# dome272/Paella

Hardware: AMD Instinct MI355X
Metric: images/sec (whole node) + single-image ms, 256x256 @ 8 steps (higher is better)
Workload: dtype f32; 1 GPU; BASELINE configs[1]: Paella 573M-class (stand-in blocks=[4,8,4]) (570.3M params), 32x32 tokens = 256 px, 8 steps, CFG 8.0, CLIP-H-text only (S=4), batch 1 per GPU, + VQGAN f8 decode; denoiser=570m, sample_steps=8, noise=philox, submission=hip-graph replay, world_size_observed=1

## Files before the change

include/paella_hip.h:

```cpp
#ifndef PAELLA_HIP_H
#define PAELLA_HIP_H

#include <stddef.h>
#include <stdint.h>

#ifdef __cplusplus
extern "C" {
#endif

#define PAELLA_ABI_VERSION 8

#define PAELLA_OK 0
#define PAELLA_ERR_ARG -1
#define PAELLA_ERR_HIP -2
#define PAELLA_ERR_WORKSPACE -3
#define PAELLA_ERR_STATE -4

#define PAELLA_MAX_LEVELS 8
#define PAELLA_MAX_BLOCK_TYPES 8

int paella_abi_version(void);
const char* paella_last_error(void);
const char* paella_source_stamp(void);

// ... 161 lines not shown
                                         const int* kw_len, int kw_pitch, const int* q_groups, int qg_pitch, const int* k_groups,
                                         int kg_pitch, const uint64_t* seeds, const float* temperature, int rows_per_sample,
                                         const int* step, const float* t_next, const int* active, const int64_t* init_noise,
                                         const int64_t* pin_keep, const int64_t* pin_tokens, const int* pin_on, int64_t* tokens_out,
                                         void* ws, size_t ws_bytes, void* stream);

int paella_sample_tail_filter(const float* logits_c, const float* logits_u, int64_t rows, int L, float cfg, float one_minus_cfg,
                              float temperature, int mode, uint64_t seed, const uint64_t* seed_ptr, uint64_t offset, int64_t row_offset,
                              const int64_t* row_offset_ptr, const int64_t* init_noise, float t_next, const int64_t* pin_keep,
                              const int64_t* pin_tokens, int top_k, float top_p, float typical_mass, int min_tokens,
                              int64_t* tokens_out, int64_t* sampled_out, void* stream);
int paella_sample_tail_stream_filter(const float* logits_c, const float* logits_u, int64_t rows, int L, const float* cfg_pairs,
                                     const float* temperature, const uint64_t* seeds, int rows_per_sample, const int* step,
                                     const float* t_next, const int* active, const int64_t* init_noise, const int64_t* pin_keep,
                                     const int64_t* pin_tokens, const int* pin_on, const int* filter_k, const float* filter_mass,
                                     int64_t* tokens_out, int64_t* sampled_out, void* stream);

int paella_sample_tail_stats(const float* logits_c, const float* logits_u, int64_t rows, int L, float cfg, float one_minus_cfg,
                             float temperature, int mode, uint64_t seed, const uint64_t* seed_ptr, uint64_t offset, int64_t row_offset,
                             const int64_t* row_offset_ptr, const int64_t* init_noise, float t_next, const int64_t* pin_keep,
                             const int64_t* pin_tokens, int top_k, float top_p, float typical_mass, int min_tokens, int64_t* tokens_out,
                             int64_t* sampled_out, float* logprob_out, float* entropy_out, void* stream);
int paella_sample_tail_stream_stats(const float* logits_c, const float* logits_u, int64_t rows, int L, const float* cfg_pairs,
                                    const float* temperature, const uint64_t* seeds, int rows_per_sample, const int* step,
                                    const float* t_next, const int* active, const int64_t* init_noise, const int64_t* pin_keep,
                                    const int64_t* pin_tokens, const int* pin_on, const int* filter_k, const float* filter_mass,
                                    int64_t* tokens_out, int64_t* sampled_out, float* logprob_out, float* entropy_out, void* stream);
int paella_renoise_select(const int64_t* drawn, const float* logprob, const int64_t* init_noise, int64_t rows, int rows_per_sample,
                          uint64_t seed, const uint64_t* seed_ptr, uint64_t offset, int64_t row_offset, const int64_t* row_offset_ptr,
                          float t_next, int policy, float confidence_noise, const int64_t* pin_keep, const int64_t* pin_tokens,
                          int64_t* tokens_out, void* stream);
int paella_renoise_select_stream(const int64_t* drawn, const float* logprob, const int64_t* init_noise, int64_t rows, int rows_per_sample,
                                 const uint64_t* seeds, const int* step, const float* t_next, const int* active, const int* policy,
                                 const float* confidence_noise, const int64_t* pin_keep, const int64_t* pin_tokens, const int* pin_on,
                                 int64_t* tokens_out, void* stream);

typedef struct paella_tail_args {
    const float *logits_c, *logits_u; int64_t rows; int32_t L;
    float cfg, one_minus_cfg, temperature; int32_t mode; uint64_t seed; const uint64_t* seed_ptr; uint64_t offset;
    int64_t row_offset; const int64_t* row_offset_ptr; float t_next; const float *noise_q, *mask_u;
    const uint64_t* seeds; const float *temperature_tab, *cfg_pairs; int32_t rows_per_sample;
    const int32_t* step; const float* t_next_tab; const int32_t* active;
    const int64_t *init_noise, *pin_keep, *pin_tokens; const int32_t* pin_on;
    int32_t top_k; float top_p, typical_mass; int32_t min_tokens; const int32_t* filter_k; const float* filter_mass;
    int64_t *tokens_out, *sampled_out; float *logprob_out, *entropy_out;
} paella_tail_args;

typedef struct paella_step_args {
    const int64_t* tokens; const float* r; const void* cond; int32_t B, n_unique; float mix_c, mix_u; const float* mix_pairs; int32_t H, W, S; const int32_t* cond_len;
    const float* attn_weights; int32_t n_attn_weights;
    const float* kw_table; const int32_t* kw_len; int32_t kw_pitch;
    const int32_t* q_groups; int32_t qg_pitch; const int32_t* k_groups; int32_t kg_pitch;
    float* logits_out; const paella_tail_args* tail;
} paella_step_args;

int paella_unet_step(paella_unet* m, const paella_step_args* args, size_t args_bytes, void* ws, size_t ws_bytes, void* stream);
int paella_sample_tail_args(const paella_tail_args* args, size_t args_bytes, void* stream);

int paella_add_noise(const int64_t* x, const float* t, const int64_t* mask_in, const int64_t* random_x,
                     const float* rand_u, uint64_t seed, uint64_t offset, int num_labels, int B,
                     int64_t per_sample, int64_t* x_out, int64_t* mask_out, void* stream);

int paella_select_tokens(const int64_t* a, const int64_t* b, const int64_t* mask, const float* flag, int64_t fill, int64_t n,
                         int64_t* out, void* stream);

typedef struct paella_vqgan paella_vqgan;
typedef struct paella_vqgan_config {
    int32_t levels, bottleneck_blocks, c_hidden, c_latent, codebook_size;
    float scale_factor;
} paella_vqgan_config;

int paella_vqgan_create(const paella_vqgan_config* cfg, paella_vqgan** out);
void paella_vqgan_destroy(paella_vqgan* v);
int paella_vqgan_load_tensor(paella_vqgan* v, const char* key, const float* dev_src, const int64_t* shape, int ndim,
                             void* stream);
int paella_vqgan_finalize(paella_vqgan* v, void* stream);
int paella_vqgan_set_precision(paella_vqgan* v, int mode, void* stream);
size_t paella_vqgan_workspace_bytes(const paella_vqgan* v, int B, int h, int w);
int paella_vqgan_decode_indices(paella_vqgan* v, const int64_t* idx, int B, int h, int w, float* img_out, void* ws,
                                size_t ws_bytes, void* stream);
int paella_vqgan_decode(paella_vqgan* v, const float* latents, int B, int h, int w, float* img_out, void* ws,
                        size_t ws_bytes, void* stream);
int paella_vqgan_encode(paella_vqgan* v, const float* img, int B, int Hp, int Wp, float* qe_out, float* x_out,
                        int64_t* idx_out, float* loss_out, void* ws, size_t ws_bytes, void* stream);
int paella_vqgan_quantize_rows(paella_vqgan* v, const float* x, int64_t rows, int64_t* idx_out, float* qe_out,
                               float* mse_out, void* stream);
int paella_vqgan_lookup_rows(paella_vqgan* v, const int64_t* idx, int64_t rows, float* out, void* stream);

int paella_op_gemm(const float* A, const float* W, const float* bias, const float* residual, float* C, int M, int N,
                   int K, int act, int tile_cfg, int splitk, void* ws, size_t ws_bytes, void* stream);
int paella_op_layernorm(const float* x, float* y, int64_t rows, int C, float eps, void* stream);
int paella_op_dwconv_ln(const float* x, const float* skip, const float* w, const float* bias, float* y, int B, int H,
                        int W, int C, float eps, void* stream);
int paella_op_grn_scale(const float* g, const float* gamma, float* scale, float* tmp, int B, int rows_per_sample,
                        int C, void* stream);
int paella_op_attention(const float* q, const float* k_self, const float* v_self, const float* k_cond,
                        const float* v_cond, float* out, int B, int nhead, int D, int Lq, int Lself, int Lcond,
                        const float* key_weights, int n_kw, void* stream);
int paella_op_attention_ragged(const float* q, const float* k_self, const float* v_self, const float* k_cond,
                               const float* v_cond, float* out, int B, int nhead, int D, int Lq, int Lself, int Lcond,
                               const int* cond_len, const float* key_weights, int n_kw, void* stream);
int paella_op_attention_kw(const float* q, const float* k_self, const float* v_self, const float* k_cond, const float* v_cond,
                           float* out, int B, int nhead, int D, int Lq, int Lself, int Lcond, const int* cond_len,
                           const float* kw_table, const int* kw_len, int kw_pitch, void* stream);
int paella_op_attention_rg(const float* q, const float* k_self, const float* v_self, const float* k_cond, const float* v_cond,
                           float* out, int B, int nhead, int D, int Lq, int Lself, int Lcond, const int* cond_len,
                           const float* kw_table, const int* kw_len, int kw_pitch, const int* q_groups, int qg_pitch,
// ... 109 lines not shown
```

paella_amd/_lib.py:

```python
import ctypes
import os
from ctypes import POINTER, Structure, c_char, c_char_p, c_double, c_float, c_int, c_int32, c_int64, c_size_t, c_uint64, c_void_p

_HERE = os.path.dirname(os.path.abspath(__file__))
LIB_PATH = os.path.join(_HERE, "csrc", "libpaella_hip.so")

MAX_LEVELS = 8
MAX_BLOCK_TYPES = 8
ABI_VERSION = 8


class UnetConfig(Structure):
    _fields_ = [
        ("c_in", c_int32), ("c_out", c_int32), ("num_labels", c_int32), ("c_r", c_int32), ("patch_size", c_int32),
        ("c_cond", c_int32), ("n_levels", c_int32),
        ("c_hidden", c_int32 * MAX_LEVELS), ("nhead", c_int32 * MAX_LEVELS), ("blocks", c_int32 * MAX_LEVELS),
        ("level_config", (c_char * MAX_BLOCK_TYPES) * MAX_LEVELS),
        ("clip_embd", c_int32), ("byt5_embd", c_int32), ("clip_seq_len", c_int32), ("kernel_size", c_int32),
        ("self_attn", c_int32),
    ]


class VqganConfig(Structure):
    _fields_ = [
        ("levels", c_int32), ("bottleneck_blocks", c_int32), ("c_hidden", c_int32), ("c_latent", c_int32),
        ("codebook_size", c_int32), ("scale_factor", c_float),
    ]


class TestGemmArgs(Structure):
    _fields_ = [
        ("A", c_void_p), ("lda", c_int), ("W", c_void_p), ("ldw", c_int), ("C", c_void_p), ("ldc", c_int),
        ("M", c_int), ("N", c_int), ("K", c_int),
        ("bias", c_void_p), ("act", c_int), ("alpha", c_float), ("residual", c_void_p), ("ldr", c_int),
        ("ts", c_void_p), ("ts_stride", c_int), ("rows_per_sample", c_int),
        ("store_mode", c_int), ("sH", c_int), ("sW", c_int), ("sC", c_int), ("py", c_int), ("px", c_int), ("n_seg_x", c_int),
        ("rowstat_out", c_void_p), ("sumsq_out", c_void_p),
        ("remap_in", c_int), ("remap_out", c_int), ("remap_off", c_int),
        ("c16", c_void_p),
        ("mode", c_int), ("scale", c_void_p), ("shift", c_void_p), ("a_rows_per_sample", c_int), ("ln_stats", c_void_p),
        ("cv_enabled", c_int), ("cv_Hi", c_int), ("cv_Wi", c_int), ("cv_C", c_int), ("cv_Ho", c_int), ("cv_Wo", c_int), ("cv_stride", c_int),
        ("cv_ntaps", c_int), ("cv_tw_log2", c_int), ("cv_oy0", c_int), ("cv_ox0", c_int), ("cv_tsign", c_int),
        ("c_capacity", c_size_t), ("c16_capacity", c_size_t), ("rowstat_capacity", c_size_t), ("sumsq_capacity", c_size_t),
    ]


class TailArgs(Structure):
    _fields_ = [
        ("logits_c", c_void_p), ("logits_u", c_void_p), ("rows", c_int64), ("L", c_int32),
        ("cfg", c_float), ("one_minus_cfg", c_float), ("temperature", c_float), ("mode", c_int32), ("seed", c_uint64), ("seed_ptr", c_void_p), ("offset", c_uint64),
        ("row_offset", c_int64), ("row_offset_ptr", c_void_p), ("t_next", c_float), ("noise_q", c_void_p), ("mask_u", c_void_p),
        ("seeds", c_void_p), ("temperature_tab", c_void_p), ("cfg_pairs", c_void_p), ("rows_per_sample", c_int32),
        ("step", c_void_p), ("t_next_tab", c_void_p), ("active", c_void_p),
        ("init_noise", c_void_p), ("pin_keep", c_void_p), ("pin_tokens", c_void_p), ("pin_on", c_void_p),
        ("top_k", c_int32), ("top_p", c_float), ("typical_mass", c_float), ("min_tokens", c_int32), ("filter_k", c_void_p), ("filter_mass", c_void_p),
        ("tokens_out", c_void_p), ("sampled_out", c_void_p), ("logprob_out", c_void_p), ("entropy_out", c_void_p),
    ]


class StepArgs(Structure):
    _fields_ = [
        ("tokens", c_void_p), ("r", c_void_p), ("cond", c_void_p), ("B", c_int32), ("n_unique", c_int32), ("mix_c", c_float), ("mix_u", c_float), ("mix_pairs", c_void_p),
        ("H", c_int32), ("W", c_int32), ("S", c_int32), ("cond_len", c_void_p),
        ("attn_weights", c_void_p), ("n_attn_weights", c_int32),
        ("kw_table", c_void_p), ("kw_len", c_void_p), ("kw_pitch", c_int32),
        ("q_groups", c_void_p), ("qg_pitch", c_int32), ("k_groups", c_void_p), ("kg_pitch", c_int32),
        ("logits_out", c_void_p), ("tail", POINTER(TailArgs)),
    ]


class AdamwTensor(Structure):
    _fields_ = [
        ("p", c_void_p), ("g", c_void_p), ("m", c_void_p), ("v", c_void_p), ("n", c_int64), ("chunk_begin", c_int64),
        ("lr", c_double), ("beta1", c_double), ("beta2", c_double), ("eps", c_double), ("weight_decay", c_double),
    ]


def tensor_fields(block, **tensors):
    for name, t in tensors.items():
        setattr(block, name, None if t is None else t.data_ptr())
    return block


SIGNATURES = {
    "paella_abi_version": (c_int, []),
    "paella_last_error": (c_char_p, []),
    "paella_source_stamp": (c_char_p, []),
    "paella_workspace_init": (c_int, [c_void_p, c_size_t, c_void_p]),
    "paella_workspace_header_bytes": (c_size_t, []),
    "paella_unet_create": (c_int, [POINTER(UnetConfig), POINTER(c_void_p)]),
    "paella_unet_destroy": (None, [c_void_p]),
    "paella_unet_load_tensor": (c_int, [c_void_p, c_char_p, c_void_p, POINTER(c_int64), c_int, c_void_p]),
    "paella_unet_set_timestep_freqs": (c_int, [c_void_p, POINTER(c_float), c_int]),
    "paella_unet_finalize": (c_int, [c_void_p, c_void_p]),
    "paella_unet_cond_bytes": (c_size_t, [c_void_p, c_int, c_int]),
    "paella_unet_workspace_bytes": (c_size_t, [c_void_p, c_int, c_int, c_int, c_int]),
    "paella_unet_cond_prepare": (c_int, [c_void_p, c_void_p, c_int, c_void_p, POINTER(c_void_p), c_int, c_int, c_void_p,
                                         c_size_t, c_void_p, c_size_t, c_void_p]),
    "paella_unet_c_embeddings": (c_int, [c_void_p, c_void_p, c_int, c_void_p, POINTER(c_void_p), c_int, c_int, c_void_p,
                                         c_void_p, c_size_t, c_void_p]),
    "paella_unet_r_embedding": (c_int, [c_void_p, c_void_p, c_int, c_float, c_void_p, c_void_p]),
    "paella_unet_forward": (c_int, [c_void_p, c_void_p, c_void_p, c_void_p, c_int, c_int, c_int, c_int, c_void_p, c_int,
                                    c_void_p, c_void_p, c_size_t, c_void_p]),
    "paella_unet_forward_shared": (c_int, [c_void_p, c_void_p, c_void_p, c_void_p, c_int, c_int, c_float, c_float, c_int, c_int, c_int,
                                           c_void_p, c_int, c_void_p, c_void_p, c_size_t, c_void_p]),
    "paella_unet_forward_sample": (c_int, [c_void_p, c_void_p, c_void_p, c_void_p, c_int, c_int, c_float, c_float, c_int, c_int, c_int,
                                           c_void_p, c_int, c_float, c_int, c_uint64, c_void_p, c_uint64, c_int64, c_void_p, c_void_p, c_float, c_void_p,
                                           c_void_p, c_size_t, c_void_p]),
    "paella_sample_tail": (c_int, [c_void_p, c_void_p, c_int64, c_int, c_float, c_float, c_float, c_int, c_void_p,
                                   c_uint64, c_uint64, c_void_p, c_void_p, c_float, c_void_p, c_void_p, c_void_p]),
    "paella_sample_tail_ex": (c_int, [c_void_p, c_void_p, c_int64, c_int, c_float, c_float, c_float, c_int, c_void_p,
                                      c_uint64, c_void_p, c_uint64, c_int64, c_void_p, c_void_p, c_void_p, c_float, c_void_p, c_void_p, c_void_p]),
    "paella_start_tokens": (c_int, [c_uint64, c_void_p, c_int64, c_void_p, c_int, c_int64, c_void_p, c_void_p]),
    "paella_sample_tail_req": (c_int, [c_void_p, c_void_p, c_int64, c_int, c_void_p, c_void_p, c_void_p, c_int, c_uint64, c_void_p, c_float, c_void_p, c_void_p,
                                       c_void_p]),
    "paella_start_tokens_req": (c_int, [c_void_p, c_int, c_int, c_int, c_void_p, c_void_p]),
    "paella_unet_forward_shared_req": (c_int, [c_void_p, c_void_p, c_void_p, c_void_p, c_int, c_int, c_void_p, c_int, c_int, c_int, c_void_p, c_int, c_void_p,
                                               c_void_p, c_size_t, c_void_p]),
    "paella_unet_forward_sample_req": (c_int, [c_void_p, c_void_p, c_void_p, c_void_p, c_int, c_int, c_void_p, c_int, c_int, c_int, c_void_p, c_int, c_void_p,
                                               c_void_p, c_int, c_uint64, c_void_p, c_float, c_void_p, c_void_p, c_size_t, c_void_p]),
    "paella_request_step": (c_int, [c_void_p, c_int, c_void_p, c_void_p, c_int, c_void_p, c_void_p, c_void_p, c_void_p, c_void_p, c_void_p, c_void_p]),
    "paella_sample_tail_stream": (c_int, [c_void_p, c_void_p, c_int64, c_int, c_void_p, c_void_p, c_void_p, c_int, c_void_p, c_void_p, c_void_p, c_void_p, c_void_p,
                                          c_void_p, c_void_p]),
    "paella_unet_forward_sample_stream": (c_int, [c_void_p, c_void_p, c_void_p, c_void_p, c_int, c_int, c_void_p, c_int, c_int, c_int, c_void_p, c_int, c_void_p,
                                                  c_void_p, c_int, c_void_p, c_void_p, c_void_p, c_void_p, c_void_p, c_void_p, c_size_t, c_void_p]),
    "paella_add_noise": (c_int, [c_void_p, c_void_p, c_void_p, c_void_p, c_void_p, c_uint64, c_uint64, c_int, c_int,
                                 c_int64, c_void_p, c_void_p, c_void_p]),
    "paella_select_tokens": (c_int, [c_void_p, c_void_p, c_void_p, c_void_p, c_int64, c_int64, c_void_p, c_void_p]),
    "paella_vqgan_create": (c_int, [POINTER(VqganConfig), POINTER(c_void_p)]),
    "paella_vqgan_destroy": (None, [c_void_p]),
    "paella_vqgan_load_tensor": (c_int, [c_void_p, c_char_p, c_void_p, POINTER(c_int64), c_int, c_void_p]),
    "paella_vqgan_finalize": (c_int, [c_void_p, c_void_p]),
    "paella_vqgan_set_precision": (c_int, [c_void_p, c_int, c_void_p]),
    "paella_vqgan_workspace_bytes": (c_size_t, [c_void_p, c_int, c_int, c_int]),
    "paella_vqgan_decode_indices": (c_int, [c_void_p, c_void_p, c_int, c_int, c_int, c_void_p, c_void_p, c_size_t, c_void_p]),
    "paella_vqgan_decode": (c_int, [c_void_p, c_void_p, c_int, c_int, c_int, c_void_p, c_void_p, c_size_t, c_void_p]),
    "paella_vqgan_encode": (c_int, [c_void_p, c_void_p, c_int, c_int, c_int, c_void_p, c_void_p, c_void_p, c_void_p,
                                    c_void_p, c_size_t, c_void_p]),
    "paella_vqgan_quantize_rows": (c_int, [c_void_p, c_void_p, c_int64, c_void_p, c_void_p, c_void_p, c_void_p]),
    "paella_vqgan_lookup_rows": (c_int, [c_void_p, c_void_p, c_int64, c_void_p, c_void_p]),
    "paella_unet_set_precision": (c_int, [c_void_p, c_int, c_void_p]),
    "paella_unet_get_precision": (c_int, [c_void_p]),
    "paella_op_gemm": (c_int, [c_void_p, c_void_p, c_void_p, c_void_p, c_void_p, c_int, c_int, c_int, c_int, c_int, c_int,
                               c_void_p, c_size_t, c_void_p]),
    "paella_op_layernorm": (c_int, [c_void_p, c_void_p, c_int64, c_int, c_float, c_void_p]),
    "paella_op_dwconv_ln": (c_int, [c_void_p, c_void_p, c_void_p, c_void_p, c_void_p, c_int, c_int, c_int, c_int, c_float,
                                    c_void_p]),
    "paella_op_grn_scale": (c_int, [c_void_p, c_void_p, c_void_p, c_void_p, c_int, c_int, c_int, c_void_p]),
    "paella_op_attention": (c_int, [c_void_p, c_void_p, c_void_p, c_void_p, c_void_p, c_void_p, c_int, c_int, c_int, c_int,
                                    c_int, c_int, c_void_p, c_int, c_void_p]),
    "paella_unet_cond_prepare_slots": (c_int, [c_void_p, c_void_p, c_int, c_void_p, POINTER(c_void_p), c_int, c_int, c_int, c_int, c_void_p,
                                               c_size_t, c_void_p, c_void_p, c_size_t, c_void_p]),
    "paella_unet_forward_shared_ragged": (c_int, [c_void_p, c_void_p, c_void_p, c_void_p, c_int, c_int, c_float, c_float, c_int, c_int, c_int, c_void_p,
                                                  c_void_p, c_int, c_void_p, c_void_p, c_size_t, c_void_p]),
# ... 86 lines not shown
    "paella_grn_act_forward_seed_dev": (c_int, [c_void_p, c_void_p, c_void_p, c_int, c_int, c_int, c_float, c_void_p, c_void_p, c_void_p, c_void_p, c_size_t, c_void_p]),
    "paella_grn_act_backward_seed_dev": (c_int, [c_void_p, c_void_p, c_void_p, c_void_p, c_int, c_int, c_int, c_float, c_void_p, c_void_p, c_void_p, c_void_p, c_void_p,
                                                 c_size_t, c_void_p]),
    "paella_attn_train_forward_seed_dev": (c_int, [c_void_p, c_int, c_void_p, c_int, c_void_p, c_int, c_int, c_int, c_int, c_int, c_int, c_float, c_void_p, c_void_p,
                                                   c_void_p, c_void_p, c_size_t, c_void_p]),
    "paella_attn_train_backward_seed_dev": (c_int, [c_void_p, c_int, c_void_p, c_int, c_void_p, c_int, c_void_p, c_void_p, c_void_p, c_int, c_int, c_int, c_int, c_int,
                                                    c_float, c_void_p, c_void_p, c_int, c_void_p, c_int, c_void_p, c_int, c_void_p, c_size_t, c_void_p]),
    "paella_embed_ln_train_workspace_bytes": (c_size_t, [c_int, c_int, c_int, c_int, c_int, c_int]),
    "paella_embed_ln_train_forward": (c_int, [c_void_p, c_void_p, c_int, c_int, c_int, c_int, c_int, c_int, c_float, c_void_p, c_void_p, c_size_t, c_void_p]),
    "paella_embed_ln_train_backward": (c_int, [c_void_p, c_void_p, c_void_p, c_int, c_int, c_int, c_int, c_int, c_int, c_float, c_void_p, c_void_p, c_size_t, c_void_p]),
}

TEST_HOOKS = {
    "paella_prof_detail": (c_int64, [c_void_p, c_void_p, c_int64]),
    "paella_prof_epi": (c_int64, [c_void_p, c_int64]),
    "paella_prof_grid": (c_int64, [c_void_p, c_int64]),
    "paella_prof_enable": (c_int, [c_int]),
    "paella_prof_collect": (c_int, [POINTER(ctypes.c_double), POINTER(ctypes.c_double), POINTER(ctypes.c_double), POINTER(c_int64)]),
    "paella_test_gemm_bf16": (c_int, [c_void_p, c_void_p, c_void_p, c_void_p, c_void_p, c_void_p, c_int, c_int, c_int, c_int, c_void_p, c_int, c_int, c_void_p, c_size_t, c_void_p]),
    "paella_test_gemm_bf16_rule": (c_int, [c_int]),
    "paella_test_grn_apply16": (c_int, [c_void_p, c_void_p, c_void_p, c_int64, c_int, c_int, c_void_p]),
    "paella_test_gemm_bf16_ln": (c_int, [c_void_p, c_void_p, c_void_p, c_void_p, c_int, c_int, c_int, c_void_p, c_int, c_int, c_void_p, c_size_t, c_void_p]),
    "paella_test_attention_bf16": (c_int, [c_void_p, c_void_p, c_void_p, c_void_p, c_void_p, c_void_p, c_int, c_int, c_int, c_int, c_int, c_int, c_void_p, c_int, c_void_p]),
    "paella_test_attention_bf16_ragged": (c_int, [c_void_p, c_void_p, c_void_p, c_void_p, c_void_p, c_void_p, c_int, c_int, c_int, c_int, c_int, c_int, c_void_p,
                                                  c_void_p, c_int, c_void_p]),
    "paella_test_attention_bf16_kw": (c_int, [c_void_p, c_void_p, c_void_p, c_void_p, c_void_p, c_void_p, c_int, c_int, c_int, c_int, c_int, c_int, c_void_p,
                                              c_void_p, c_void_p, c_int, c_void_p]),
    "paella_test_launch_chain": (c_int, [c_void_p, c_int, c_int, c_int, c_void_p]),
    "paella_test_attention_variant": (c_int, [c_int]),
    "paella_test_gemm_dma": (c_int, [c_int]),
    "paella_test_gemm_epi_specialise": (c_int, [c_int]),
    "paella_test_gemm_raster": (c_int, [c_int]),
    "paella_test_gemm_ring": (c_int, [c_int]),
    "paella_test_ring_resident": (ctypes.c_long, [c_int, c_int]),
    "paella_test_gemm_site": (c_int, [c_int, c_int, c_int, c_int, c_int, c_int]),
    "paella_test_gemm_site_cfg": (c_int, [c_int, c_int, c_int, c_int, c_int, c_int, c_int]),
    "paella_test_gemm_big_stagger": (c_int, [c_int]),
    "paella_test_grn_fuse": (c_int, [c_int]),
    "paella_test_ln_fold_ratio": (c_int, [c_float]),
    "paella_test_ln_guard_counter": (c_int, [c_void_p]),
    "paella_test_mlp_grn_fused": (c_int, [c_void_p] * 10 + [c_int, c_int, c_int, c_void_p, c_size_t, c_void_p]),
    "paella_test_gemm_tail_tile": (c_int, [c_int]),
    "paella_test_tail_scores": (c_int, [c_void_p, c_void_p, c_int64, c_int, c_float, c_float, c_float, c_uint64, c_uint64, c_int64, c_void_p, c_void_p]),
    "paella_test_tail_scores_req": (c_int, [c_void_p, c_void_p, c_int64, c_int, c_void_p, c_void_p, c_void_p, c_int, c_uint64, c_void_p, c_void_p]),
    "paella_test_tail_filter_keep": (c_int, [c_void_p, c_void_p, c_int64, c_int, c_float, c_float, c_float, c_int, c_float, c_float, c_int, c_void_p, c_void_p, c_void_p,
                                             c_int, c_void_p, c_void_p, c_void_p, c_void_p, c_void_p]),
    "paella_test_renoise_scores": (c_int, [c_void_p, c_void_p, c_void_p, c_int64, c_int, c_uint64, c_uint64, c_int64, c_float, c_int, c_float, c_void_p, c_void_p, c_void_p,
                                           c_void_p, c_void_p, c_void_p, c_void_p, c_void_p, c_void_p, c_void_p, c_void_p, c_void_p]),
    "paella_test_gemm_prologue": (c_int, [c_void_p, c_void_p, c_void_p, c_int, c_int, c_int, c_int, c_void_p, c_void_p, c_int, c_void_p, c_int, c_int,
                                          c_void_p, c_size_t, c_void_p]),
    "paella_test_gemm_desc": (c_int, [POINTER(TestGemmArgs), c_int, c_int, c_void_p, c_size_t, c_void_p]),
    "paella_test_gemm_args_size": (c_size_t, []),
    "paella_test_embed_ln_unshuffle": (c_int, [c_void_p, c_void_p, c_void_p, c_int, c_int, c_int, c_int, c_int, c_int, c_float, c_void_p]),
}

_lib = None


class PaellaHipError(RuntimeError):
    pass


def load():
    global _lib
    if _lib is not None:
        return _lib
    if not os.path.exists(LIB_PATH):
        raise PaellaHipError(
            "libpaella_hip.so is not built (%s). Run `python -m paella_amd.build` (needs hipcc); "
            "paella_amd has no non-HIP fallback." % LIB_PATH)
    try:
        lib = ctypes.CDLL(LIB_PATH)
    except OSError as e:
        raise PaellaHipError("cannot load %s: %s" % (LIB_PATH, e)) from e
    for name, (res, args) in list(SIGNATURES.items()) + list(TEST_HOOKS.items()):
        fn = getattr(lib, name)
        fn.restype = res
        fn.argtypes = args
    from ._stamp import source_stamp
    try:
        here = source_stamp()
    except OSError as e:
        raise PaellaHipError("cannot verify %s: the kernel sources it is checked against are missing (%s)" % (LIB_PATH, e)) from e
    built = lib.paella_source_stamp().decode()
    if built != here:
        raise PaellaHipError("libpaella_hip.so was built from other sources (library stamp %s, sources in the tree %s): rebuild with "
                             "`python -m paella_amd.build`; a stale library is never used silently" % (built, here))
    if lib.paella_abi_version() != ABI_VERSION:
        raise PaellaHipError("libpaella_hip.so ABI %d != binding ABI %d" % (lib.paella_abi_version(), ABI_VERSION))
    _lib = lib
    return lib


def check(rc):
    if rc != 0:
        msg = load().paella_last_error()
        raise PaellaHipError("libpaella_hip error %d: %s" % (rc, msg.decode("utf-8", "replace") if msg else "?"))


def ptr(t):
    return None if t is None else c_void_p(t.data_ptr())


def new_workspace(nbytes, device):
    import torch
    lib = load()
# ... 11 lines not shown
```

paella_amd/csrc/common.h:

```cpp
#pragma once
#include <hip/hip_runtime.h>
#include <stdint.h>
#include <stddef.h>

typedef float f32x4 __attribute__((ext_vector_type(4)));

#define PAELLA_OK 0
#define PAELLA_ERR_ARG -1
#define PAELLA_ERR_HIP -2
#define PAELLA_ERR_WORKSPACE -3
#define PAELLA_ERR_STATE -4

void paella_set_error(const char* fmt, ...);

#define HIP_CHECK_RET(expr)                                                          \
    do {                                                                             \
        hipError_t _e = (expr);                                                      \
        if (_e != hipSuccess) {                                                      \
            paella_set_error("%s:%d: %s -> %s", __FILE__, __LINE__, #expr,           \
                             hipGetErrorString(_e));                                 \
            return PAELLA_ERR_HIP;                                                   \
        }                                                                            \
    } while (0)

// ... 89 lines not shown
    int Hi, Wi, C, Ho, Wo, stride, ntaps;
    int tw_log2, oy0, ox0, tsign;
};

struct GemmArgs {
    const float* A; int lda;
    const float* W; int ldw;
    float* C; int ldc;
    int M, N, K;
    const float* a_scale;
    const float* a_shift;
    int a_rows_per_sample;
    FastDiv a_rps_div;
    const float* grn_gx;
    const float* grn_gamma;
    const float* grn_part;
    int grn_np;
    int force_ring_cfg;
    const float* ln_stats;
    int ln_nblk;
    float ln_eps;
    const float* ln_row;
    float ln_fold_ratio;
    const float* ln_wsum;
    unsigned* ln_guard_count;
    Epilogue ep;
    FusedTail ft;
    ConvGather cv;
    const unsigned short* A16;
    const unsigned short* W16;
    ReqTables rq;
};

struct TailArgs;
static const size_t kGemmMaxTickets = (size_t)1 << 16;
static const size_t kGemmTicketBytes = kGemmMaxTickets * sizeof(unsigned);
int launch_gemm(const GemmArgs& g, void* ws, size_t ws_bytes, hipStream_t stream);
int launch_gemm_cfg(const GemmArgs& g, int cfg, int splitk, void* ws, size_t ws_bytes, hipStream_t stream);
int gemm_num_tile_configs();
int gemm_grn_fused_tile(int M, int C4, int C, int rows_per_sample, bool allow_64);
int gemm_tail_tiles_n(int M, int N, bool bf16_operands = false);
int launch_gemm_tail(const GemmArgs& g, hipStream_t stream);
int gemm_tail_config(int M, int N, bool bf16_operands = false);
int launch_tail_finalize(const TailArgs& a, const float* part_score, const int* part_idx, int tiles_n, hipStream_t stream);
static inline bool gemm_bf16_ok(int K, int lda, int ldw) { return K > 0 && (K & 63) == 0 && (lda & 7) == 0 && (ldw & 7) == 0; }

int launch_ln_rowstat_finalize(const float* stats, int nblk, int K, float eps, float* out4, int64_t M, const float* A32, unsigned short* A16, int lda, float ratio,
                               unsigned* guard_count, hipStream_t stream);

int launch_layernorm(const float* x, float* y, int64_t rows, int C, float eps, float g_mul, float g_add,
                     int s2d, int H, int W, hipStream_t stream);
int launch_layernorm16(const float* x, float* y, unsigned short* y16, int64_t rows, int C, float eps, float g_mul, float g_add,
                       int s2d, int H, int W, hipStream_t stream);
int launch_grn_apply16(unsigned short* h, const float* scale, const float* shift, int64_t rows, int rows_per_sample, int C, hipStream_t stream);
int launch_grn_partials_apply16(const float* part, const float* gamma, const float* shift, float* scale, unsigned short* h, int B, int rows_per_sample, int C, hipStream_t stream);
int launch_f32_to_bf16(const float* src, unsigned short* dst, size_t n, hipStream_t stream);
int launch_rowsum_bf16(const unsigned short* W, float* out, int N, int K, hipStream_t stream);

int launch_dwconv_ln(const float* x, const float* skip, const float* w, const float* bias, float* y,
                     int B, int H, int W, int C, float eps, hipStream_t stream, unsigned short* y16 = nullptr);
int launch_dwconv_res(const float* x, const float* xt, const float* w, const float* bias, float* y,
                      int B, int H, int W, int C, float gamma2, hipStream_t stream);

int launch_grn_scale(const float* g, const float* gamma, float* scale, float* tmp_gx, int B,
                     int rows_per_sample, int C, hipStream_t stream);

int launch_grn_from_partials(const float* part, const float* gamma, float* scale, int B, int groups, int C, hipStream_t stream);

int launch_embed_ln_unshuffle(const int64_t* tokens, const float* table, float* out, int B, int H, int W,
                              int c_in, int patch, int num_labels, float eps, hipStream_t stream);

int launch_timestep(const float* r, const float* freqs, const float* Wcat, const float* bcat, float* ts,
                    int B, int c_r, int total, float max_positions, float* r_embed_out, int reps, hipStream_t stream);
int launch_scale_shift(float* x, const float* ts, int ts_stride, int64_t rows, int rows_per_sample, int C,
                       hipStream_t stream);

int launch_silu(const float* x, float* y, int64_t n, hipStream_t stream);
int launch_copy_rows(const float* src, int lds, float* dst, int ldd, int64_t rows, int cols, hipStream_t stream);
int launch_axpby(float* x, const float* y, float a, float b, int64_t n, hipStream_t stream);
int launch_axpby16(float* x, const float* y, float a, float b, int64_t n, unsigned short* x16, hipStream_t stream);
int launch_axpby16_req(float* x, const float* y, const float* ab, int B, int64_t per_sample, unsigned short* x16, hipStream_t stream);

struct AttnArgs {
    const float* q; int ldq;
    const float* k_self; const float* v_self; int ld_self;
    const float* k_cond; const float* v_cond; int ld_cond;
    float* out; int ldo;
    int B, nhead, D, Lq, Lself, Lcond;
    float scale;
    const float* key_weights;
    int n_kw;
    unsigned short* out16;
    const unsigned short* q16; const unsigned short* k_self16; const unsigned short* v_self16; int ld16;
    const int* cond_len;
    const float* kw_table = nullptr;
    const int* kw_len = nullptr;
    int kw_pitch = 0;
    const int* q_groups = nullptr;
    const int* k_groups = nullptr;
    int qg_pitch = 0, kg_pitch = 0;
};
int launch_attention(const AttnArgs& a, hipStream_t stream);

struct TailArgs {
    const float* logits_c; const float* logits_u;
    int64_t rows; int L;
    float cfg, one_minus_cfg, temperature;
    int mode;
    const float* noise_q;
    uint64_t seed; uint64_t offset;
    int64_t row_offset;
    const uint64_t* seed_ptr;
    const int64_t* row_offset_ptr;
    const int64_t* init_noise;
    const float* mask_u;
    float t_next;
    int64_t* tokens_out;
    int64_t* sampled_out;
    ReqTables rq;
    const int64_t* pin_keep = nullptr;
    const int64_t* pin_tokens = nullptr;
    const int* pin_on = nullptr;
};
int launch_sample_tail(const TailArgs& a, hipStream_t stream);
struct TailFilter {
    int top_k = 0, min_tokens = 1;
    float top_p = 1.f, typical_mass = 1.f;
    const int* filter_k = nullptr;
    const float* filter_mass = nullptr;
    unsigned char* keep_out = nullptr;
    float* rec_out = nullptr;
// ... 42 lines not shown
```

paella_amd/csrc/elementwise.hip:

```cpp
#include "common.h"
#include "gemm_device.h"

#define WAVES_PER_BLOCK 4

__device__ __forceinline__ float wave_sum(float v) {
#pragma unroll
    for (int o = 32; o > 0; o >>= 1) v += __shfl_xor(v, o, 64);
    return v;
}

__device__ __forceinline__ f32x4 ld4(const float* p) { return *reinterpret_cast<const f32x4*>(p); }
__device__ __forceinline__ void st4(float* p, f32x4 v) { *reinterpret_cast<f32x4*>(p) = v; }
__device__ __forceinline__ float hsum4(f32x4 v) { return (v[0] + v[1]) + (v[2] + v[3]); }
typedef __bf16 bf16x4 __attribute__((ext_vector_type(4)));
typedef __bf16 bf16x8 __attribute__((ext_vector_type(8)));
typedef float f32x8 __attribute__((ext_vector_type(8)));
__device__ __forceinline__ void st4h(unsigned short* p, f32x4 v) { *reinterpret_cast<bf16x4*>(p) = __builtin_convertvector(v, bf16x4); }

template <int NV>
__device__ __forceinline__ void ln_regs(f32x4 (&v)[NV], int C4, int lane, int C, float eps, float mul, float add) {
    float s = 0.f;
#pragma unroll
    for (int i = 0; i < NV; ++i)
        if (lane + i * 64 < C4) s += hsum4(v[i]);
// ... 29 lines not shown
    }
    ln_regs<NV>(v, C4, lane, C, eps, g_mul, g_add);
    int64_t yo;
    if (s2d) {
        const int64_t hw = (int64_t)H * W;
        const int64_t b = row / hw;
        const int rem = (int)(row - b * hw);
        const int yy = rem / W, xx = rem - yy * W;
        const int64_t orow = (b * (H >> 1) + (yy >> 1)) * (W >> 1) + (xx >> 1);
        yo = orow * (4 * (int64_t)C) + ((yy & 1) * 2 + (xx & 1)) * C;
    } else {
        yo = row * C;
    }
    if (y16) {
#pragma unroll
        for (int i = 0; i < NV; ++i) {
            const int c4 = lane + i * 64;
            if (c4 < C4) st4h(y16 + yo + c4 * 4, v[i]);
        }
    }
    if (y) {
#pragma unroll
        for (int i = 0; i < NV; ++i) {
            const int c4 = lane + i * 64;
            if (c4 < C4) st4(y + yo + c4 * 4, v[i]);
        }
    }
}

#define DISPATCH_NV(C4, ...)                                                       \
    do {                                                                           \
        const int _nv = ((C4) + 63) / 64;                                          \
        if (_nv <= 1) { constexpr int NV = 1; __VA_ARGS__; }                       \
        else if (_nv <= 2) { constexpr int NV = 2; __VA_ARGS__; }                  \
        else if (_nv <= 3) { constexpr int NV = 3; __VA_ARGS__; }                  \
        else if (_nv <= 5) { constexpr int NV = 5; __VA_ARGS__; }                  \
        else if (_nv <= 8) { constexpr int NV = 8; __VA_ARGS__; }                  \
        else if (_nv <= 16) { constexpr int NV = 16; __VA_ARGS__; }                \
        else { paella_set_error("channel count %d too large", (C4) * 4); return PAELLA_ERR_ARG; } \
    } while (0)

int launch_layernorm(const float* x, float* y, int64_t rows, int C, float eps, float g_mul, float g_add, int s2d,
                     int H, int W, hipStream_t st) {
    return launch_layernorm16(x, y, nullptr, rows, C, eps, g_mul, g_add, s2d, H, W, st);
}
int launch_layernorm16(const float* x, float* y, unsigned short* y16, int64_t rows, int C, float eps, float g_mul, float g_add, int s2d,
                       int H, int W, hipStream_t st) {
    if (rows <= 0) return PAELLA_OK;
    if (C & 3) { paella_set_error("layernorm: C %% 4 != 0 (C=%d)", C); return PAELLA_ERR_ARG; }
    if (s2d && ((H & 1) || (W & 1))) { paella_set_error("layernorm s2d: odd grid %dx%d", H, W); return PAELLA_ERR_ARG; }
    const unsigned blocks = (unsigned)((rows + WAVES_PER_BLOCK - 1) / WAVES_PER_BLOCK);
    DISPATCH_NV(C >> 2, hipLaunchKernelGGL((layernorm_kernel<NV>), dim3(blocks), dim3(64 * WAVES_PER_BLOCK), 0, st, x, y, y16,
                                           rows, C, eps, g_mul, g_add, s2d, H, W));
    LAUNCH_CHECK_RET();
    return PAELLA_OK;
}

__global__ __launch_bounds__(256) void ln_rowstat_finalize_kernel(const float* __restrict__ stats, int nblk, int K, float eps, f32x4* __restrict__ out, int64_t M,
                                                                  const float* __restrict__ A32, unsigned short* __restrict__ A16, int lda, float ratio,
                                                                  unsigned* __restrict__ guard_count) {
    const int64_t row = (int64_t)blockIdx.x * 16 + (threadIdx.x >> 4);
    const int l16 = threadIdx.x & 15;
    if (row >= M) return;
    const float* st = stats + (size_t)row * nblk * 2;
    RowStatAcc acc;
    for (int j = l16; j < nblk; j += 16) acc.add(st[2 * j], st[2 * j + 1]);
#pragma unroll
    for (int o = 1; o < 16; o <<= 1) { acc.S += __shfl_xor(acc.S, o, 64); acc.Q += __shfl_xor(acc.Q, o, 64); acc.M += __shfl_xor(acc.M, o, 64); }
    float mu, rs;
    acc.finish(K, eps, mu, rs);
    const float mu_lo = (float)(acc.S / (double)K - (double)mu);
    if (l16 == 0) out[row] = f32x4{mu, rs, mu_lo, fabsf(mu) * rs};
    if (A16 && fabsf(mu) * rs > ratio) {
        typedef __bf16 bf16x4_t __attribute__((ext_vector_type(4)));
        const float* src = A32 + (size_t)row * lda;
        unsigned short* dst = A16 + (size_t)row * lda;
        for (int k = l16 * 4; k < K; k += 64) {
            f32x4 v = *reinterpret_cast<const f32x4*>(src + k);
#pragma unroll
            for (int e = 0; e < 4; ++e) v[e] = ((v[e] - mu) - mu_lo) * rs;
            *reinterpret_cast<bf16x4_t*>(dst + k) = __builtin_convertvector(v, bf16x4_t);
        }
        if (guard_count && l16 == 0) atomicAdd(guard_count, 1u);
    }
}

int launch_ln_rowstat_finalize(const float* stats, int nblk, int K, float eps, float* out4, int64_t M, const float* A32, unsigned short* A16, int lda, float ratio,
                               unsigned* guard_count, hipStream_t st) {
    if (M <= 0) return PAELLA_OK;
    if (A16 && (!A32 || (K & 3) || (lda & 3))) { paella_set_error("ln_rowstat_finalize: the bf16 rewrite needs the fp32 rows and K, lda %% 4 == 0"); return PAELLA_ERR_ARG; }
    hipLaunchKernelGGL(ln_rowstat_finalize_kernel, dim3((unsigned)((M + 15) / 16)), dim3(256), 0, st, stats, nblk, K, eps, reinterpret_cast<f32x4*>(out4), M, A32, A16, lda, ratio,
                       guard_count);
    LAUNCH_CHECK_RET();
    return PAELLA_OK;
}


template <int NV>
__global__ __launch_bounds__(64 * WAVES_PER_BLOCK) void dwconv_res_kernel(const float* __restrict__ x,
                                                                         const float* __restrict__ xt,
                                                                         const float* __restrict__ w,
                                                                         const float* __restrict__ bias,
                                                                         float* __restrict__ y, int B, int H, int W, int C,
                                                                         float gamma2) {
    const int lane = threadIdx.x & 63;
    const int64_t pos = (int64_t)blockIdx.x * WAVES_PER_BLOCK + (threadIdx.x >> 6);
    const int64_t total = (int64_t)B * H * W;
    if (pos >= total) return;
    const int C4 = C >> 2;
    const int xx = (int)(pos % W);
    const int yy = (int)((pos / W) % H);
    const int64_t base = pos - (int64_t)yy * W - xx;
    f32x4 acc[NV];
#pragma unroll
    for (int i = 0; i < NV; ++i) {
        const int c4 = lane + i * 64;
        acc[i] = c4 < C4 ? ld4(bias + c4 * 4) : f32x4{0.f, 0.f, 0.f, 0.f};
    }
#pragma unroll
    for (int ky = 0; ky < 3; ++ky) {
        const int sy = min(max(yy + ky - 1, 0), H - 1);
#pragma unroll
        for (int kx = 0; kx < 3; ++kx) {
            const int sx = min(max(xx + kx - 1, 0), W - 1);
            const int64_t npos = base + (int64_t)sy * W + sx;
            const int tap = ky * 3 + kx;
#pragma unroll
            for (int i = 0; i < NV; ++i) {
                const int c4 = lane + i * 64;
                if (c4 < C4) acc[i] += ld4(xt + npos * C + c4 * 4) * ld4(w + tap * C + c4 * 4);
            }
        }
    }
#pragma unroll
    for (int i = 0; i < NV; ++i) {
        const int c4 = lane + i * 64;
        if (c4 < C4) st4(y + pos * C + c4 * 4, ld4(x + pos * C + c4 * 4) + acc[i] * gamma2);
    }
}

int launch_dwconv_res(const float* x, const float* xt, const float* w, const float* bias, float* y, int B, int H,
                      int W, int C, float gamma2, hipStream_t st) {
    const int64_t total = (int64_t)B * H * W;
    if (total <= 0) return PAELLA_OK;
    if (C & 3) { paella_set_error("dwconv_res: C %% 4 != 0"); return PAELLA_ERR_ARG; }
    const unsigned blocks = (unsigned)((total + WAVES_PER_BLOCK - 1) / WAVES_PER_BLOCK);
    DISPATCH_NV(C >> 2, hipLaunchKernelGGL((dwconv_res_kernel<NV>), dim3(blocks), dim3(64 * WAVES_PER_BLOCK), 0, st, x, xt, w,
                                           bias, y, B, H, W, C, gamma2));
    LAUNCH_CHECK_RET();
    return PAELLA_OK;
}

__global__ __launch_bounds__(256) void grn_sumsq_kernel(const float* __restrict__ g, float* __restrict__ gx, int rows_per_sample,
                                                        int C) {
    __shared__ float red[4][64];
    const int cl = threadIdx.x & 63, rg = threadIdx.x >> 6;
    const int c = blockIdx.x * 64 + cl;
    const int b = blockIdx.y;
    float s = 0.f;
    if (c < C) {
        const float* p = g + ((size_t)b * rows_per_sample) * C + c;
        for (int r = rg; r < rows_per_sample; r += 4) {
            const float v = p[(size_t)r * C];
            s += v * v;
        }
    }
    red[rg][cl] = s;
    __syncthreads();
    if (rg == 0 && c < C) gx[(size_t)b * C + c] = sqrtf((red[0][cl] + red[1][cl]) + (red[2][cl] + red[3][cl]));
}

__global__ __launch_bounds__(256) void grn_finalize_kernel(const float* __restrict__ gx, const float* __restrict__ gamma,
                                                           float* __restrict__ scale, int C) {
    __shared__ float red[256];
    const int b = blockIdx.x;
    const float* p = gx + (size_t)b * C;
    float s = 0.f;
    for (int c = threadIdx.x; c < C; c += 256) s += p[c];
    red[threadIdx.x] = s;
    __syncthreads();
    for (int o = 128; o > 0; o >>= 1) {
        if ((int)threadIdx.x < o) red[threadIdx.x] += red[threadIdx.x + o];
        __syncthreads();
    }
    const float denom = red[0] / (float)C + 1e-6f;
    for (int c = threadIdx.x; c < C; c += 256) scale[(size_t)b * C + c] = 1.0f + gamma[c] * (p[c] / denom);
}

template <int G>
__global__ __launch_bounds__(1024) void grn_from_partials_kernel(const float* __restrict__ part, const float* __restrict__ gamma,
                                                                 float* __restrict__ scale, int groups_rt, int C) {
    __shared__ float red[16];
    const int groups = G > 0 ? G : groups_rt;
    const int b = blockIdx.y;
    const int C4 = C >> 2;
    const float* p = part + (size_t)b * groups * C;
    auto colsum = [&](int c4) {
        f32x4 q = f32x4{0.f, 0.f, 0.f, 0.f};
        if (G > 0) {
            f32x4 v[G > 0 ? G : 1];
#pragma unroll
            for (int g = 0; g < G; ++g) v[g] = ld4(p + (size_t)g * C + c4 * 4);
#pragma unroll
            for (int g = 0; g < G; ++g) q += v[g];
        } else {
// ... 69 lines not shown
#pragma unroll
    for (int t = 0; t < P * P; ++t) {
        const int dy = t / P, dx = t % P;
        int64_t tok = tokens[(b * H + (oy * P + dy)) * W + (ox * P + dx)];
        tok = tok < 0 ? 0 : (tok >= num_labels ? num_labels - 1 : tok);
        const float* row = table + tok * c_in;
        float s = 0.f;
        for (int c4 = lane; c4 < C4; c4 += 64) s += hsum4(ld4(row + c4 * 4));
        const float mean = wave_sum(s) / (float)c_in;
        float q = 0.f;
        for (int c4 = lane; c4 < C4; c4 += 64) {
            f32x4 d = ld4(row + c4 * 4) - mean;
            d = d * d;
            q += hsum4(d);
        }
        const float rstd = 1.0f / sqrtf(wave_sum(q) / (float)c_in + eps);
        for (int c4 = lane; c4 < C4; c4 += 64) {
            const f32x4 n = (ld4(row + c4 * 4) - mean) * rstd;
#pragma unroll
            for (int e = 0; e < 4; ++e) orow[(c4 * 4 + e) * (P * P) + t] = n[e];
        }
    }
}

int launch_embed_ln_unshuffle(const int64_t* tokens, const float* table, float* out, int B, int H, int W, int c_in,
                              int patch, int num_labels, float eps, hipStream_t st) {
    if (c_in & 3) { paella_set_error("embed: c_in %% 4 != 0"); return PAELLA_ERR_ARG; }
    if (patch < 1 || patch > 2 || (H % patch) || (W % patch)) {
        paella_set_error("embed: unsupported patch_size %d for grid %dx%d (supported: 1, 2)", patch, H, W);
        return PAELLA_ERR_ARG;
    }
    const int64_t total = (int64_t)B * (H / patch) * (W / patch);
    if (total <= 0) return PAELLA_OK;
    if (total > 0x7fffffff) { paella_set_error("embed: too many positions"); return PAELLA_ERR_ARG; }
    const unsigned blocks = (unsigned)((total + WAVES_PER_BLOCK - 1) / WAVES_PER_BLOCK);
    const FastDiv dWo = fast_div_of((unsigned)(W / patch)), dHo = fast_div_of((unsigned)(H / patch));
    if (patch == 2)
        hipLaunchKernelGGL((embed_ln_unshuffle_kernel<2>), dim3(blocks), dim3(64 * WAVES_PER_BLOCK), 0, st, tokens, table, out,
                           B, H, W, c_in, num_labels, eps, dWo, dHo);
    else
        hipLaunchKernelGGL((embed_ln_unshuffle_kernel<1>), dim3(blocks), dim3(64 * WAVES_PER_BLOCK), 0, st, tokens, table, out,
                           B, H, W, c_in, num_labels, eps, dWo, dHo);
    LAUNCH_CHECK_RET();
    return PAELLA_OK;
}

__global__ __launch_bounds__(256) void timestep_kernel(const float* __restrict__ r, const float* __restrict__ freqs,
                                                       const float* __restrict__ Wcat, const float* __restrict__ bcat,
                                                       float* __restrict__ ts, int c_r, int total, float max_positions,
                                                       float* __restrict__ r_embed_out, int reps, int n_distinct) {
    extern __shared__ float emb[];
    const int b = blockIdx.y;
    const int half = c_r >> 1;
    const float rr = r[b] * max_positions;
    for (int k = threadIdx.x; k < c_r; k += 256) {
        float v = 0.f;
        if (k < half) v = sinf(rr * freqs[k]);
        else if (k < 2 * half) v = cosf(rr * freqs[k - half]);
        emb[k] = v;
        if (r_embed_out && blockIdx.x == 0) r_embed_out[(size_t)b * c_r + k] = v;
    }
    __syncthreads();
    const int o = blockIdx.x * 256 + threadIdx.x;
    if (o >= total) return;
    const float* w = Wcat + (size_t)o * c_r;
    float acc = 0.f;
    for (int k = 0; k < c_r; ++k) acc += emb[k] * w[k];
    const float out = acc + bcat[o];
    for (int rep = 0; rep < reps; ++rep) ts[((size_t)rep * n_distinct + b) * total + o] = out;
}

int launch_timestep(const float* r, const float* freqs, const float* Wcat, const float* bcat, float* ts, int B,
                    int c_r, int total, float max_positions, float* r_embed_out, int reps, hipStream_t st) {
    if (B <= 0) return PAELLA_OK;
    int gx = (total + 255) / 256;
    if (gx < 1) gx = 1;
    hipLaunchKernelGGL(timestep_kernel, dim3(gx, B), dim3(256), c_r * sizeof(float), st, r, freqs, Wcat, bcat, ts, c_r,
                       total, max_positions, r_embed_out, reps < 1 ? 1 : reps, B);
    LAUNCH_CHECK_RET();
    return PAELLA_OK;
}

__global__ __launch_bounds__(256) void scale_shift_kernel(float* __restrict__ x, const float* __restrict__ ts, int ts_stride,
                                                          int64_t rows, int rows_per_sample, int C) {
    const int C4 = C >> 2;
    const int64_t total = rows * C4;
    for (int64_t i = (int64_t)blockIdx.x * 256 + threadIdx.x; i < total; i += (int64_t)gridDim.x * 256) {
        const int64_t row = i / C4;
        const int c = (int)(i - row * C4) * 4;
        const float* t = ts + (row / rows_per_sample) * ts_stride;
        const f32x4 v = ld4(x + row * C + c);
        st4(x + row * C + c, v * (1.0f + ld4(t + c)) + ld4(t + C + c));
    }
}

int launch_scale_shift(float* x, const float* ts, int ts_stride, int64_t rows, int rows_per_sample, int C,
                       hipStream_t st) {
    if (rows <= 0) return PAELLA_OK;
    if (C & 3) { paella_set_error("scale_shift: C %% 4 != 0"); return PAELLA_ERR_ARG; }
    int64_t blocks = (rows * (C >> 2) + 255) / 256;
    if (blocks > 4096) blocks = 4096;
    hipLaunchKernelGGL(scale_shift_kernel, dim3((unsigned)blocks), dim3(256), 0, st, x, ts, ts_stride, rows, rows_per_sample, C);
    LAUNCH_CHECK_RET();
    return PAELLA_OK;
}

__global__ __launch_bounds__(256) void silu_kernel(const float* __restrict__ x, float* __restrict__ y, int64_t n) {
    for (int64_t i = (int64_t)blockIdx.x * 256 + threadIdx.x; i < n; i += (int64_t)gridDim.x * 256) {
        const float v = x[i];
        y[i] = v / (1.0f + expf(-v));
    }
}
int launch_silu(const float* x, float* y, int64_t n, hipStream_t st) {
    if (n <= 0) return PAELLA_OK;
    int64_t blocks = (n + 255) / 256;
    if (blocks > 4096) blocks = 4096;
    hipLaunchKernelGGL(silu_kernel, dim3((unsigned)blocks), dim3(256), 0, st, x, y, n);
    LAUNCH_CHECK_RET();
    return PAELLA_OK;
}

__global__ __launch_bounds__(256) void copy_rows_kernel(const float* __restrict__ src, int lds_, float* __restrict__ dst, int ldd,
                                                        int64_t rows, int cols) {
    const int64_t total = rows * cols;
    for (int64_t i = (int64_t)blockIdx.x * 256 + threadIdx.x; i < total; i += (int64_t)gridDim.x * 256) {
        const int64_t r = i / cols;
        const int c = (int)(i - r * cols);
        dst[r * ldd + c] = src[r * lds_ + c];
    }
}
__global__ __launch_bounds__(256) void copy_rows4_kernel(const float* __restrict__ src, int lds_, float* __restrict__ dst, int ldd, unsigned total4, int cols4, FastDiv dC) {
    for (unsigned i = blockIdx.x * 256u + threadIdx.x; i < total4; i += gridDim.x * 256u) {
        const unsigned r = fast_div(i, dC);
        const unsigned c = (i - r * (unsigned)cols4) * 4u;
        st4(dst + (size_t)r * ldd + c, ld4(src + (size_t)r * lds_ + c));
    }
}
__global__ __launch_bounds__(256) void axpby_kernel(float* __restrict__ x, const float* __restrict__ y, float a, float b, int64_t n4, unsigned short* __restrict__ x16) {
    for (int64_t i = (int64_t)blockIdx.x * 256 + threadIdx.x; i < n4; i += (int64_t)gridDim.x * 256) {
        const f32x4 v = ld4(x + i * 4) * a + ld4(y + i * 4) * b;
        st4(x + i * 4, v);
        if (x16) st4h(x16 + i * 4, v);
    }
}
__global__ __launch_bounds__(256) void axpby_req_kernel(float* __restrict__ x, const float* __restrict__ y, const float* __restrict__ ab, int64_t per4, unsigned short* __restrict__ x16) {
    const int s = blockIdx.y;
    const float a = ab[2 * s], b = ab[2 * s + 1];
    for (int64_t j = (int64_t)blockIdx.x * 256 + threadIdx.x; j < per4; j += (int64_t)gridDim.x * 256) {
        const int64_t i = (int64_t)s * per4 + j;
        const f32x4 v = ld4(x + i * 4) * a + ld4(y + i * 4) * b;
        st4(x + i * 4, v);
        if (x16) st4h(x16 + i * 4, v);
    }
}
int launch_axpby16_req(float* x, const float* y, const float* ab, int B, int64_t per_sample, unsigned short* x16, hipStream_t st) {
    if (B <= 0 || per_sample <= 0) return PAELLA_OK;
    if (!ab || (per_sample & 3) || B > 65535) { paella_set_error("axpby_req: needs a pair table, per_sample %% 4 == 0 and at most 65535 samples"); return PAELLA_ERR_ARG; }
    int64_t blocks = (per_sample / 4 + 255) / 256;
    if (blocks > 1024) blocks = 1024;
    hipLaunchKernelGGL(axpby_req_kernel, dim3((unsigned)blocks, (unsigned)B), dim3(256), 0, st, x, y, ab, per_sample / 4, x16);
    LAUNCH_CHECK_RET();
    return PAELLA_OK;
}
int launch_axpby(float* x, const float* y, float a, float b, int64_t n, hipStream_t st) { return launch_axpby16(x, y, a, b, n, nullptr, st); }
int launch_axpby16(float* x, const float* y, float a, float b, int64_t n, unsigned short* x16, hipStream_t st) {
    if (n <= 0) return PAELLA_OK;
    if (n & 3) { paella_set_error("axpby: n %% 4 != 0"); return PAELLA_ERR_ARG; }
    int64_t blocks = (n / 4 + 255) / 256;
    if (blocks > 8192) blocks = 8192;
    hipLaunchKernelGGL(axpby_kernel, dim3((unsigned)blocks), dim3(256), 0, st, x, y, a, b, n / 4, x16);
    LAUNCH_CHECK_RET();
    return PAELLA_OK;
}

int launch_copy_rows(const float* src, int lds_, float* dst, int ldd, int64_t rows, int cols, hipStream_t st) {
    if (rows <= 0 || cols <= 0) return PAELLA_OK;
    if (!((cols | lds_ | ldd) & 3) && !(((uintptr_t)src | (uintptr_t)dst) & 15) && rows * (cols / 4) < 0x7fffffff) {
        const int64_t total4 = rows * (cols / 4);
        int64_t blocks4 = (total4 + 255) / 256;
        if (blocks4 > 4096) blocks4 = 4096;
        hipLaunchKernelGGL(copy_rows4_kernel, dim3((unsigned)blocks4), dim3(256), 0, st, src, lds_, dst, ldd, (unsigned)total4, cols / 4, fast_div_of((unsigned)(cols / 4)));
        LAUNCH_CHECK_RET();
        return PAELLA_OK;
    }
    int64_t blocks = (rows * cols + 255) / 256;
    if (blocks > 4096) blocks = 4096;
    hipLaunchKernelGGL(copy_rows_kernel, dim3((unsigned)blocks), dim3(256), 0, st, src, lds_, dst, ldd, rows, cols);
    LAUNCH_CHECK_RET();
    return PAELLA_OK;
}

__global__ __launch_bounds__(256) void grn_apply16_kernel(unsigned short* __restrict__ h, const float* __restrict__ scale, const float* __restrict__ shift,
                                                          unsigned total8, int C8, FastDiv dC8, FastDiv dRps) {
    for (unsigned i = blockIdx.x * 256u + threadIdx.x; i < total8; i += gridDim.x * 256u) {
        const unsigned row = fast_div(i, dC8);
        const unsigned c = (i - row * (unsigned)C8) * 8u;
        const unsigned b = fast_div(row, dRps);
        const bf16x8 v = *reinterpret_cast<const bf16x8*>(h + (size_t)i * 8);
        const float* sp = scale + (size_t)b * ((size_t)C8 * 8) + c;
        const f32x4 s0 = ld4(sp), s1 = ld4(sp + 4), t0 = ld4(shift + c), t1 = ld4(shift + c + 4);
        const f32x8 f = __builtin_convertvector(v, f32x8);
        f32x8 o;
#pragma unroll
        for (int e = 0; e < 4; ++e) { o[e] = f[e] * s0[e] + t0[e]; o[4 + e] = f[4 + e] * s1[e] + t1[e]; }
        *reinterpret_cast<bf16x8*>(h + (size_t)i * 8) = __builtin_convertvector(o, bf16x8);
    }
}
__global__ __launch_bounds__(256) void grn_apply16_cols_kernel(unsigned short* __restrict__ h, const float* __restrict__ scale, const float* __restrict__ shift, int C, int rows_per_sample) {
    const int c = (blockIdx.x * 64 + (threadIdx.x & 63)) * 8;
    const int b = blockIdx.z;
    const int r0 = blockIdx.y * 16 + (threadIdx.x >> 6);
    unsigned short* hp = h + ((size_t)b * rows_per_sample + r0) * C + c;
    bf16x8 v[4];
#pragma unroll
    for (int k = 0; k < 4; ++k) v[k] = *reinterpret_cast<const bf16x8*>(hp + (size_t)(4 * k) * C);
    const float* sp = scale + (size_t)b * C + c;
    const f32x4 s0 = ld4(sp), s1 = ld4(sp + 4), t0 = ld4(shift + c), t1 = ld4(shift + c + 4);
#pragma unroll
    for (int k = 0; k < 4; ++k) {
        const f32x8 f = __builtin_convertvector(v[k], f32x8);
        f32x8 o;
#pragma unroll
        for (int e = 0; e < 4; ++e) { o[e] = f[e] * s0[e] + t0[e]; o[4 + e] = f[4 + e] * s1[e] + t1[e]; }
// ... 128 lines not shown
```

paella_amd/csrc/model.hip:

```cpp
#include "internal.h"
#include "test_hooks.h"
#include "../../include/paella_hip.h"

#include <math.h>
#include <stdarg.h>
#include <stdio.h>
#include <string.h>

#include <map>
#include <string>
#include <vector>

static thread_local char g_err[2048] = "";
void paella_set_error(const char* fmt, ...) {
    va_list ap;
    va_start(ap, fmt);
    vsnprintf(g_err, sizeof(g_err), fmt, ap);
    va_end(ap);
}
extern "C" const char* paella_last_error(void) { return g_err; }
extern "C" int paella_abi_version(void) { return PAELLA_ABI_VERSION; }

int devbuf_alloc(DevBuf& b, size_t n) {
    if (b.p && b.n == n) return PAELLA_OK;
    if (b.p) { (void)hipFree(b.p); b.p = nullptr; }
    b.n = n;
    HIP_CHECK_RET(hipMalloc((void**)&b.p, (n ? n : 1) * sizeof(float)));
    return PAELLA_OK;
}

enum BlockType { BT_RES, BT_TS, BT_ATTN, BT_FF, BT_DOWN, BT_UP };

struct Block {
    BlockType type;
    int level = 0;
    int c = 0;
    bool has_skip = false;
    int ts_offset = -1;
    bool ts_standalone = true;
    int fused_ts = -1;
    int attn_index = -1;
    bool emit_rowstat = false;
    bool ln_from_stats = false;
    int c_from = 0, c_to = 0;
    Weight *dw_w = nullptr, *dw_b = nullptr;
    Weight *w1 = nullptr, *b1 = nullptr, *gamma = nullptr, *beta = nullptr, *w2 = nullptr, *b2 = nullptr;
    Weight *in_w = nullptr, *in_b = nullptr, *out_w = nullptr, *out_b = nullptr, *kv_w = nullptr, *kv_b = nullptr;
    Weight *conv_w = nullptr, *conv_b = nullptr;
};

struct LnWeight { Weight* t; int N, K; };

struct paella_unet {
    paella_unet_config cfg;
    std::vector<Block> down, up;
    std::map<std::string, Weight> t;
    Weight *byt5_w, *byt5_b, *clip_w, *clip_b, *clip_image_w, *clip_image_b;
    Weight *in_mapper, *embedding_w, *embedding_b, *clf_w, *clf_b, *out_mapper;
    std::vector<Weight*> shadowed;
    std::vector<LnWeight> ln_weights;
    DevBuf ts_w, ts_b, freqs;
// ... 473 lines not shown
    carve_forward(m, a, B, H, W, S, f);
    Arena c(nullptr, 0);
    carve_cond(m, c, B, S, f);
    return (a.off > c.off ? a.off : c.off) + 256;
}

static int compute_c_embed(const paella_unet* m, const float* byt5, int S_byt5, const float* clip, const float* const* clip_image,
                           int n_clip_image, int B, int S, float* c_embed, float* splitk, hipStream_t st) {
    const paella_unet_config& c = m->cfg;
    const size_t skb = kSplitKBudget;
    const int cc = c.c_cond;
    if (S_byt5 > 0) {
        GemmArgs g = gemm_args(byt5, c.byt5_embd, m->byt5_w->w.p, c.byt5_embd, c_embed, cc, B * S_byt5, cc, c.byt5_embd);
        g.ep.bias = m->byt5_b->w.p;
        g.ep.remap_in = S_byt5; g.ep.remap_out = S; g.ep.remap_off = 0;
        RET_IF(launch_gemm(g, splitk, skb, st));
    }
    int row_off = S_byt5;
    if (clip) {
        GemmArgs g = gemm_args(clip, c.clip_embd, m->clip_w->w.p, c.clip_embd, c_embed + (size_t)row_off * cc, S * cc, B,
                               cc * c.clip_seq_len, c.clip_embd);
        g.ep.bias = m->clip_b->w.p;
        RET_IF(launch_gemm(g, splitk, skb, st));
        row_off += c.clip_seq_len;
    }
    for (int i = 0; i < n_clip_image; ++i) {
        if (!clip_image || !clip_image[i]) { paella_set_error("clip_image[%d] is null", i); return PAELLA_ERR_ARG; }
        GemmArgs g = gemm_args(clip_image[i], c.clip_embd, m->clip_image_w->w.p, c.clip_embd,
                               c_embed + (size_t)row_off * cc, S * cc, B, cc * c.clip_seq_len, c.clip_embd);
        g.ep.bias = m->clip_image_b->w.p;
        RET_IF(launch_gemm(g, splitk, skb, st));
        row_off += c.clip_seq_len;
    }
    RET_IF(launch_layernorm(c_embed, c_embed, (int64_t)B * S, cc, 1e-6f, 1.f, 0.f, 0, 0, 0, st));
    return PAELLA_OK;
}

extern "C" int paella_unet_c_embeddings(paella_unet* m, const float* byt5, int S_byt5, const float* clip,
                                        const float* const* clip_image, int n_clip_image, int B, float* c_embed_out, void* ws,
                                        size_t ws_bytes, void* stream) {
    if (!m || !m->finalized) { paella_set_error("model not finalized"); return PAELLA_ERR_STATE; }
    const int S = S_byt5 + (clip ? m->cfg.clip_seq_len : 0) + n_clip_image * m->cfg.clip_seq_len;
    if (B <= 0 || S <= 0 || !c_embed_out) { paella_set_error("bad conditioning shape"); return PAELLA_ERR_ARG; }
    if (ws_bytes < kSplitKBudget || !ws) { paella_set_error("workspace too small"); return PAELLA_ERR_WORKSPACE; }
    return compute_c_embed(m, byt5, S_byt5, clip, clip_image, n_clip_image, B, S, c_embed_out, (float*)ws, (hipStream_t)stream);
}

extern "C" int paella_unet_r_embedding(paella_unet* m, const float* r, int B, float max_positions, float* r_embed_out, void* stream) {
    if (!m || !m->finalized) { paella_set_error("model not finalized"); return PAELLA_ERR_STATE; }
    if (!r || !r_embed_out) { paella_set_error("null argument"); return PAELLA_ERR_ARG; }
    return launch_timestep(r, m->freqs.p, m->ts_w.p, m->ts_b.p, nullptr, B, m->cfg.c_r, 0, max_positions, r_embed_out, 1, (hipStream_t)stream);
}

static int cond_prepare_impl(paella_unet* m, const float* byt5, int S_byt5, const float* clip, const float* const* clip_image, int n_clip_image, int B,
                             int S_slot, int slot0, void* cond_out, size_t cond_bytes, int* cond_len, void* ws, size_t ws_bytes, void* stream) {
    if (!m || !m->finalized) { paella_set_error("model not finalized"); return PAELLA_ERR_STATE; }
    hipStream_t st = (hipStream_t)stream;
    const paella_unet_config& c = m->cfg;
    const int S = S_byt5 + (clip ? c.clip_seq_len : 0) + n_clip_image * c.clip_seq_len;
    if (B <= 0 || S_byt5 < 0 || n_clip_image < 0) { paella_set_error("bad conditioning shape"); return PAELLA_ERR_ARG; }
    const bool slots = S_slot > 0;
    if (slots && (slot0 < 0 || S > S_slot || !cond_len)) {
        paella_set_error("cond_prepare_slots: %d conditioning rows do not fit a slot of %d rows (or slot0 < 0 / cond_len is null)", S, S_slot);
        return PAELLA_ERR_ARG;
    }
    if (S <= 0 && (slots || m->n_attn > 0)) { paella_set_error("conditioning sequence is empty"); return PAELLA_ERR_ARG; }
    if (slots) HIP_CHECK_RET(hipMemsetD32Async((hipDeviceptr_t)(cond_len + slot0), S, (size_t)B, st));
    if (m->n_attn == 0) return PAELLA_OK;
    if (S_byt5 > 0 && !byt5) { paella_set_error("byt5 is null"); return PAELLA_ERR_ARG; }
    const size_t need = slots ? (size_t)(slot0 + B) * S_slot * (size_t)m->kv_total * sizeof(float) : paella_unet_cond_bytes(m, B, S);
    if (cond_bytes < need || !cond_out) { paella_set_error("cond buffer too small"); return PAELLA_ERR_WORKSPACE; }
    FwdBuffers f;
    Arena a(ws, ws_bytes);
    carve_cond(m, a, B, S, f);
    if (!a.ok || !ws) { paella_set_error("workspace too small (%zu needed)", a.off); return PAELLA_ERR_WORKSPACE; }
    const size_t skb = kSplitKBudget;

    const int cc = c.c_cond;
    RET_IF(compute_c_embed(m, byt5, S_byt5, clip, clip_image, n_clip_image, B, S, f.c_embed, f.splitk, st));
    RET_IF(launch_silu(f.c_embed, f.c_silu, (int64_t)B * S * cc, st));

    GemmArgs g = gemm_args(f.c_silu, cc, m->kv_w.p, cc, (float*)cond_out, m->kv_total, B * S, m->kv_total, cc);
    g.ep.bias = m->kv_b.p;
    if (slots) { g.ep.remap_in = S; g.ep.remap_out = S_slot; g.ep.remap_off = slot0 * S_slot; }
    RET_IF(launch_gemm(g, f.splitk, skb, st));
    return PAELLA_OK;
}

extern "C" int paella_unet_cond_prepare(paella_unet* m, const float* byt5, int S_byt5, const float* clip,
                                        const float* const* clip_image, int n_clip_image, int B, void* cond_out,
                                        size_t cond_bytes, void* ws, size_t ws_bytes, void* stream) {
    return cond_prepare_impl(m, byt5, S_byt5, clip, clip_image, n_clip_image, B, 0, 0, cond_out, cond_bytes, nullptr, ws, ws_bytes, stream);
}

extern "C" int paella_unet_cond_prepare_slots(paella_unet* m, const float* byt5, int S_byt5, const float* clip, const float* const* clip_image,
                                              int n_clip_image, int B, int S_slot, int slot0, void* cache, size_t cache_bytes, int* cond_len, void* ws,
                                              size_t ws_bytes, void* stream) {
    if (S_slot <= 0) { paella_set_error("cond_prepare_slots: S_slot must be > 0"); return PAELLA_ERR_ARG; }
    return cond_prepare_impl(m, byt5, S_byt5, clip, clip_image, n_clip_image, B, S_slot, slot0, cache, cache_bytes, cond_len, ws, ws_bytes, stream);
}

struct FwdCtx {
    const paella_unet* m;
    const paella_step_args& s;
    hipStream_t st;
    FwdBuffers f;
// ... 137 lines not shown

static int unet_query_total(const paella_unet* m, int H, int W) {
    const int p = m->cfg.patch_size;
    int tot = 0;
    for (int l = 0; l < m->cfg.n_levels; ++l) tot += ((H / p) >> l) * ((W / p) >> l);
    return tot;
}
static int rg_table_check(const char* who, const paella_unet* m, const paella_step_args& s) {
    if (!s.q_groups && !s.k_groups) return PAELLA_OK;
    if (!s.q_groups || !s.k_groups) { paella_set_error("%s: q_groups and k_groups must be given together (one key-group table without the other)", who); return PAELLA_ERR_ARG; }
    if (s.kg_pitch < s.S || s.qg_pitch < 1) { paella_set_error("%s: key-group pitches too small (kg_pitch %d < S %d, or qg_pitch %d < 1)", who, s.kg_pitch, s.S, s.qg_pitch); return PAELLA_ERR_ARG; }
    if (!m) { paella_set_error("%s: null model", who); return PAELLA_ERR_ARG; }
    if (m->precision == 1) { paella_set_error("%s: the key-group tables are not offered in the bf16 precision mode", who); return PAELLA_ERR_ARG; }
    const int p = m->cfg.patch_size, div = p << (m->cfg.n_levels - 1);
    if (s.H <= 0 || s.W <= 0 || s.H % div || s.W % div) { paella_set_error("%s: token grid %dx%d must be a positive multiple of %d", who, s.H, s.W, div); return PAELLA_ERR_ARG; }
    if (s.qg_pitch < unet_query_total(m, s.H, s.W)) {
        paella_set_error("%s: qg_pitch %d smaller than the %d queries of all levels of a %dx%d grid", who, s.qg_pitch, unet_query_total(m, s.H, s.W), s.H, s.W);
        return PAELLA_ERR_ARG;
    }
    return PAELLA_OK;
}

static int unet_forward_impl(paella_unet* m, const paella_step_args& s, const TailArgs* tail, void* ws, size_t ws_bytes, void* stream) {
    if (!m || !m->finalized) { paella_set_error("model not finalized"); return PAELLA_ERR_STATE; }
    if (!s.tokens || !s.r || (!s.logits_out && !tail)) { paella_set_error("null argument"); return PAELLA_ERR_ARG; }
    const paella_unet_config& c = m->cfg;
    const int p = c.patch_size;
    const int div = p << (c.n_levels - 1);
    const int H = s.H, W = s.W, n_unique = s.n_unique;
    int B = s.B;
    if (B <= 0 || H <= 0 || W <= 0 || H % div || W % div) {
        paella_set_error("token grid %dx%d must be a positive multiple of %d", H, W, div);
        return PAELLA_ERR_ARG;
    }
    if (m->n_attn > 0 && (!s.cond || s.S <= 0)) { paella_set_error("conditioning cache missing"); return PAELLA_ERR_ARG; }
    FwdCtx cx = {m, s, (hipStream_t)stream, {}, B};
    Arena a(ws, ws_bytes);
    carve_forward(m, a, B, H, W, s.S, cx.f);
    if (!a.ok || !ws) { paella_set_error("workspace too small (%zu needed, %zu given)", a.off, ws_bytes); return PAELLA_ERR_WORKSPACE; }
    hipStream_t st = cx.st;
    FwdBuffers& f = cx.f;
    int split = -1;
    for (size_t i = 0; i < m->down.size(); ++i)
        if (m->down[i].type == BT_ATTN) { split = (int)i; break; }
    if (n_unique <= 0 || n_unique > B || B % n_unique) { paella_set_error("n_unique must divide B"); return PAELLA_ERR_ARG; }
    const bool mix = s.mix_pairs || s.mix_c != 0.f || s.mix_u != 0.f;
    if (mix && B != 2 * n_unique) { paella_set_error("guidance mix needs B == 2 * n_unique"); return PAELLA_ERR_ARG; }
    const int Bfull = B;
    if (n_unique < B) {
        if (split < 0) split = 0;
        B = n_unique; cx.B = n_unique;
    }

    if (m->ts_total > 0)
        RET_IF(launch_timestep(s.r, m->freqs.p, m->ts_w.p, m->ts_b.p, f.ts, B, c.c_r, m->ts_total, 10000.0f, f.remb, Bfull / B, st));

    const int h0 = H / p, w0 = W / p;
    const int64_t n0 = (int64_t)B * h0 * w0;
    RET_IF(launch_embed_ln_unshuffle(s.tokens, m->in_mapper->w.p, f.h, B, H, W, c.c_in, p, c.num_labels, 1e-6f, st));
    {
        GemmArgs g = gemm_args(f.h, c.c_in * p * p, m->embedding_w->w.p, c.c_in * p * p, f.g, c.c_hidden[0], (int)n0, c.c_hidden[0], c.c_in * p * p);
        g.ep.bias = m->embedding_b->w.p;
        RET_IF(launch_gemm(g, f.splitk, kSplitKBudget, st));
        RET_IF(launch_layernorm(f.g, f.xl[0], n0, c.c_hidden[0], 1e-6f, 1.f, 0.f, 0, 0, 0, st));
    }

    float* x = f.xl[0];
    int h = h0, w = w0;
    for (size_t bi = 0; bi < m->down.size(); ++bi) {
        const Block& b = m->down[bi];
        if ((int)bi == split && B != Bfull) {
            const int reps = Bfull / B;
            int lvl = 0;
            for (size_t j = 0; j < bi; ++j) if (m->down[j].type == BT_DOWN) lvl = m->down[j].level;
            for (int rep = 1; rep < reps; ++rep) {
                for (int l = 0; l <= lvl; ++l) {
                    const int64_t rows_l = (int64_t)B * (h0 >> l) * (w0 >> l);
                    const int cl = c.c_hidden[l];
                    RET_IF(launch_copy_rows(f.xl[l], cl, f.xl[l] + (size_t)rep * rows_l * cl, cl, rows_l, cl, st));
                }
                const int64_t rows_c = (int64_t)B * h * w;
                const int sc = c.c_hidden[lvl] / 16 * 2;
                if (f.rowstat && c.c_hidden[lvl] % 16 == 0)
                    RET_IF(launch_copy_rows(f.rowstat, sc, f.rowstat + (size_t)rep * rows_c * sc, sc, rows_c, sc, st));
                if (f.x16 && c.c_hidden[lvl] % 8 == 0) {
                    const int c2 = c.c_hidden[lvl] / 2;
                    RET_IF(launch_copy_rows(reinterpret_cast<const float*>(f.x16), c2, reinterpret_cast<float*>(f.x16) + (size_t)rep * rows_c * c2, c2, rows_c, c2, st));
                }
            }
            B = Bfull; cx.B = Bfull;
        }
        switch (b.type) {
            case BT_DOWN: {
                const int64_t rows_in = (int64_t)B * h * w;
                const unsigned short* const w16 = ((4 * b.c_from) % 64) == 0 ? W16(m, b.conv_w) : nullptr;
                GemmArgs g = gemm_args(f.h, 4 * b.c_from, b.conv_w->w.p, 4 * b.c_from, f.xl[b.level], b.c_to, (int)(rows_in / 4), b.c_to, 4 * b.c_from);
                RET_IF(ln_operand(cx, g, b.conv_w, w16, false, x, rows_in, b.c_from, 1, h, w));
                h >>= 1; w >>= 1;
                g.ep.bias = b.conv_b->w.p;
                RET_IF(launch_gemm(g, f.splitk, kSplitKBudget, st));
                x = f.xl[b.level];
                break;
            }
            case BT_RES: case BT_FF: RET_IF(run_mlp_block(cx, b, x, nullptr, h, w)); break;
            case BT_ATTN: RET_IF(run_attn_block(cx, b, x, h, w)); break;
            case BT_TS:
                if (b.ts_standalone)
                    RET_IF(launch_scale_shift(x, f.ts + b.ts_offset, m->ts_total, (int64_t)B * h * w, h * w, b.c, st));
                break;
            default: break;
        }
    }
    if (B != Bfull) { paella_set_error("internal: shared prefix never diverged"); return PAELLA_ERR_STATE; }
    for (const Block& b : m->up) {
        switch (b.type) {
            case BT_UP: {
                const int64_t rows_in = (int64_t)B * h * w;
                float* dst = f.xu[b.level - 1];
                GemmArgs g = gemm_args(f.h, b.c_from, b.conv_w->w.p, b.c_from, dst, b.c_to, (int)rows_in, 4 * b.c_to, b.c_from);
                const unsigned short* const w16 = (b.c_from % 64) == 0 ? W16(m, b.conv_w) : nullptr;
                RET_IF(ln_operand(cx, g, b.conv_w, w16, b.ln_from_stats, x, rows_in, b.c_from));
                g.ep.bias = b.conv_b->w.p;
                g.ep.store_mode = STORE_D2S; g.ep.sH = h; g.ep.sW = w; g.ep.sC = b.c_to; g.ep.n_seg_x = 2;
                RET_IF(launch_gemm(g, f.splitk, kSplitKBudget, st));
                h <<= 1; w <<= 1;
                x = dst;
                break;
            }
            case BT_RES: case BT_FF: RET_IF(run_mlp_block(cx, b, x, b.has_skip ? f.xl[b.level] : nullptr, h, w)); break;
            case BT_ATTN: RET_IF(run_attn_block(cx, b, x, h, w)); break;
            case BT_TS:
                if (b.ts_standalone)
                    RET_IF(launch_scale_shift(x, f.ts + b.ts_offset, m->ts_total, (int64_t)B * h * w, h * w, b.c, st));
                break;
            default: break;
        }
    }
    {
        const int p2 = p * p;
        const int64_t n0 = (int64_t)B * h0 * w0;
        GemmArgs g = gemm_args(f.h, c.c_hidden[0], m->clf_w->w.p, c.c_hidden[0], f.g, c.c_out, (int)n0, c.c_out * p2, c.c_hidden[0]);
        const unsigned short* const wc16 = (c.c_hidden[0] % 64) == 0 ? W16(m, m->clf_w) : nullptr;
        RET_IF(ln_operand(cx, g, m->clf_w, wc16, m->clf_from_stats, x, n0, c.c_hidden[0]));
        g.ep.bias = m->clf_b->w.p;
        if (p == 2) { g.ep.store_mode = STORE_D2S; g.ep.sH = h0; g.ep.sW = w0; g.ep.sC = c.c_out; g.ep.n_seg_x = 2; }
        RET_IF(launch_gemm(g, f.splitk, kSplitKBudget, st));
        int64_t nt = (int64_t)B * H * W;
        const unsigned short* const wh16 = (c.c_out % 64) == 0 ? W16(m, m->out_mapper) : nullptr;
        if (wh16 && !mix) RET_IF(launch_layernorm16(f.g, nullptr, f.h16, nt, c.c_out, 1e-6f, 1.f, 0.f, 0, 0, 0, st));
        else RET_IF(launch_layernorm(f.g, f.h, nt, c.c_out, 1e-6f, 1.f, 0.f, 0, 0, 0, st));
        if (mix) {
            nt /= 2;
            if (s.mix_pairs) RET_IF(launch_axpby16_req(f.h, f.h + (size_t)nt * c.c_out, s.mix_pairs, n_unique, (int64_t)H * W * c.c_out, wh16 ? f.h16 : nullptr, st));
            else RET_IF(launch_axpby16(f.h, f.h + (size_t)nt * c.c_out, s.mix_c, s.mix_u, nt * c.c_out, wh16 ? f.h16 : nullptr, st));
        }
        GemmArgs go = gemm_args(f.h, c.c_out, m->out_mapper->w.p, c.c_out, tail ? nullptr : s.logits_out, c.num_labels, (int)nt, c.num_labels, c.c_out);
        if (wh16) { go.A16 = f.h16; go.W16 = wh16; }
        if (!tail) {
            RET_IF(launch_gemm_cfg(go, gemm_tail_config((int)nt, c.num_labels, wh16 != nullptr), 1, f.splitk, kSplitKBudget, st));
        } else {
            const int tn = gemm_tail_tiles_n((int)nt, c.num_labels, wh16 != nullptr);
            if (tn > (c.num_labels + 63) / 64) { paella_set_error("internal: fused tail tiles narrower than 64 labels (tiles_n=%d)", tn); return PAELLA_ERR_STATE; }
            if (tail->rows != nt || tail->L != c.num_labels) { paella_set_error("fused tail: row / label count mismatch"); return PAELLA_ERR_ARG; }
            go.C = nullptr;
            go.ft.temperature = tail->temperature; go.ft.mode = tail->mode; go.ft.seed = tail->seed; go.ft.seed_ptr = tail->seed_ptr;
            go.ft.offset = tail->offset; go.ft.row_offset = tail->row_offset; go.ft.row_offset_ptr = tail->row_offset_ptr;
            go.rq = tail->rq;
            go.ft.part_score = f.g;
            go.ft.part_idx = reinterpret_cast<int*>(f.g + (size_t)nt * tn);
            RET_IF(launch_gemm_tail(go, st));
            RET_IF(launch_tail_finalize(*tail, go.ft.part_score, go.ft.part_idx, tn, st));
        }
    }
    return PAELLA_OK;
}

static int run_step_block(const char* who, paella_unet* m, const paella_step_args& s, int need, void* ws, size_t ws_bytes, void* stream) {
    if ((!s.tail && !s.logits_out) || ((need & kNeedPairs) && !s.mix_pairs)) { paella_set_error("%s: null argument (logits_out / mix_pairs)", who); return PAELLA_ERR_ARG; }
    if (s.mix_pairs && (s.mix_c != 0.f || s.mix_u != 0.f)) { paella_set_error("%s: a guidance pair table and a scalar mix exclude each other", who); return PAELLA_ERR_ARG; }
    if (s.kw_len && (!s.kw_table || s.kw_pitch < 1)) { paella_set_error("%s: kw_len needs kw_table and kw_pitch >= 1", who); return PAELLA_ERR_ARG; }
    if (s.kw_len && s.attn_weights) { paella_set_error("%s: one attn_weights vector and the key-weight table exclude each other", who); return PAELLA_ERR_ARG; }
    RET_IF(rg_table_check(who, m, s));
    TailArgs a;
    if (s.tail) {
        TailFilter f;
        TailStats st;
        int kind = 0;
        RET_IF(tail_block_convert(who, *s.tail, need, true, a, f, st, &kind));
        const bool mix = s.mix_pairs || s.mix_c != 0.f || s.mix_u != 0.f;
        if (!mix && s.n_unique != s.B) {
            paella_set_error("%s without a guidance mix needs n_unique == B (separate cond / uncond logits take the unfused path)", who);
            return PAELLA_ERR_ARG;
        }
        if (a.rq.rows_per_sample > 0 && (s.H <= 0 || s.W <= 0 || a.rq.rows_per_sample != s.H * s.W)) {
            paella_set_error("%s: rows_per_sample (%d) must equal H * W", who, a.rq.rows_per_sample);
            return PAELLA_ERR_ARG;
        }
        a.rows = (int64_t)(mix ? s.n_unique : s.B) * s.H * s.W;
        a.L = m ? m->cfg.num_labels : 0;
    }
    return unet_forward_impl(m, s, s.tail ? &a : nullptr, ws, ws_bytes, stream);
}

extern "C" int paella_unet_step(paella_unet* m, const paella_step_args* args, size_t args_bytes, void* ws, size_t ws_bytes, void* stream) {
// ... 279 lines not shown
    e.store_mode = a->store_mode; e.sH = a->sH; e.sW = a->sW; e.sC = a->sC; e.py = a->py; e.px = a->px; e.n_seg_x = a->n_seg_x;
    e.rowstat_out = a->rowstat_out; e.sumsq_out = a->sumsq_out;
    e.remap_in = a->remap_in; e.remap_out = a->remap_out; e.remap_off = a->remap_off;
    e.c16 = a->c16;
    if (a->cv_enabled) {
        g.cv.enabled = 1; g.cv.Hi = a->cv_Hi; g.cv.Wi = a->cv_Wi; g.cv.C = a->cv_C; g.cv.Ho = a->cv_Ho; g.cv.Wo = a->cv_Wo; g.cv.stride = a->cv_stride; g.cv.ntaps = a->cv_ntaps;
        g.cv.tw_log2 = a->cv_tw_log2; g.cv.oy0 = a->cv_oy0; g.cv.ox0 = a->cv_ox0; g.cv.tsign = a->cv_tsign;
    }
    RET_IF(test_gemm_set_prologue(g, a->mode, a->scale, a->shift, a->a_rows_per_sample, a->ln_stats, (hipStream_t)stream));
    return launch_gemm_cfg(g, tile_cfg, splitk, ws, ws_bytes, (hipStream_t)stream);
}
extern "C" int paella_test_mlp_grn_fused(const float* h, const float* W1, const float* b1, const float* gamma, const float* beta, const float* W2,
                                         float* hidden, float* gx, float* part, float* out, int M, int c, int rps, void* ws, size_t ws_bytes, void* stream) {
    const int tile = (rps % 16 == 0) ? gemm_grn_fused_tile(M, 4 * c, c, rps, true) : 0;
    if (!tile) { paella_set_error("fused GRN not applicable (M=%d c=%d rows per sample=%d)", M, c, rps); return PAELLA_ERR_ARG; }
    hipStream_t st = (hipStream_t)stream;
    const int np = (4 * c / 32) * 2;
    GemmArgs g1 = gemm_args(h, c, W1, c, hidden, 4 * c, M, 4 * c, c);
    g1.ep.bias = b1; g1.ep.act = ACT_GELU;
    g1.ep.grn_gx_out = gx; g1.ep.grn_part_out = part; g1.ep.grn_rps = rps; g1.ep.grn_np = np;
    g1.force_ring_cfg = tile;
    RET_IF(launch_gemm(g1, ws, ws_bytes, st));
    GemmArgs g2 = gemm_args(hidden, 4 * c, W2, 4 * c, out, c, M, c, 4 * c);
    g2.grn_gx = gx; g2.grn_part = part; g2.grn_np = np; g2.grn_gamma = gamma; g2.a_shift = beta; g2.a_rows_per_sample = rps;
    return launch_gemm(g2, ws, ws_bytes, st);
}
extern "C" int paella_test_gemm_bf16(const unsigned short* A16, const unsigned short* W16, const float* bias, const float* residual, float* C, unsigned short* C16,
                                     int M, int N, int K, int act, const float* ln_stats, int tile_cfg, int splitk, void* ws, size_t ws_bytes, void* stream) {
    GemmArgs g = gemm_args(nullptr, K, nullptr, K, C, N, M, N, K);
    g.A16 = A16; g.W16 = W16;
    g.ep.bias = bias; g.ep.act = act; g.ep.residual = residual; g.ep.ldr = N; g.ep.c16 = C16;
    if (ln_stats) {
        static DevBuf wsum;
        if (wsum.n < (size_t)N) RET_IF(devbuf_alloc(wsum, (size_t)N));
        RET_IF(launch_rowsum_bf16(W16, wsum.p, N, K, (hipStream_t)stream));
        g.ln_stats = ln_stats; g.ln_nblk = K / 16; g.ln_eps = 1e-6f; g.ln_wsum = wsum.p;
    }
    return launch_gemm_cfg(g, tile_cfg, splitk, ws, ws_bytes, (hipStream_t)stream);
}
extern "C" int paella_test_gemm_bf16_ln(const unsigned short* A16, const float* A32, const unsigned short* W16, float* C, int M, int N, int K, const float* ln_stats,
                                        int tile_cfg, int splitk, void* ws, size_t ws_bytes, void* stream) {
    if (!ln_stats) { paella_set_error("gemm_bf16_ln: statistics required"); return PAELLA_ERR_ARG; }
    GemmArgs g = gemm_args(A32, K, nullptr, K, C, N, M, N, K);
    g.A16 = A16; g.W16 = W16;
    static DevBuf wsum;
    if (wsum.n < (size_t)N) RET_IF(devbuf_alloc(wsum, (size_t)N));
    RET_IF(launch_rowsum_bf16(W16, wsum.p, N, K, (hipStream_t)stream));
    g.ln_stats = ln_stats; g.ln_nblk = K / 16; g.ln_eps = 1e-6f; g.ln_wsum = wsum.p;
    return launch_gemm_cfg(g, tile_cfg, splitk, ws, ws_bytes, (hipStream_t)stream);
}
extern "C" int paella_test_grn_apply16(unsigned short* h, const float* scale, const float* shift, int64_t rows, int rows_per_sample, int C, void* stream) {
    return launch_grn_apply16(h, scale, shift, rows, rows_per_sample, C, (hipStream_t)stream);
}
extern "C" int paella_op_layernorm(const float* x, float* y, int64_t rows, int C, float eps, void* stream) {
    return launch_layernorm(x, y, rows, C, eps, 1.f, 0.f, 0, 0, 0, (hipStream_t)stream);
}
extern "C" int paella_op_dwconv_ln(const float* x, const float* skip, const float* w, const float* bias, float* y, int B, int H, int W,
                                   int C, float eps, void* stream) {
    return launch_dwconv_ln(x, skip, w, bias, y, B, H, W, C, eps, (hipStream_t)stream);
}
extern "C" int paella_op_grn_scale(const float* g, const float* gamma, float* scale, float* tmp, int B, int rows_per_sample, int C,
                                   void* stream) {
    return launch_grn_scale(g, gamma, scale, tmp, B, rows_per_sample, C, (hipStream_t)stream);
}
static int op_attention_impl(const float* q, const float* k_self, const float* v_self, const float* k_cond, const float* v_cond, float* out, int B, int nhead, int D,
                             int Lq, int Lself, int Lcond, const int* cond_len, const float* key_weights, int n_kw, const float* kw_table, const int* kw_len,
                             int kw_pitch, const int* q_groups, int qg_pitch, const int* k_groups, int kg_pitch, void* stream) {
    AttnArgs a;
    const int ld = nhead * D;
    a.q = q; a.ldq = ld; a.k_self = k_self; a.v_self = v_self; a.ld_self = ld; a.k_cond = k_cond; a.v_cond = v_cond; a.ld_cond = ld;
    a.out = out; a.ldo = ld; a.B = B; a.nhead = nhead; a.D = D; a.Lq = Lq; a.Lself = Lself; a.Lcond = Lcond;
    a.scale = 1.0f / sqrtf((float)D); a.key_weights = key_weights; a.n_kw = key_weights ? n_kw : 0; a.out16 = nullptr;
    a.q16 = nullptr; a.k_self16 = nullptr; a.v_self16 = nullptr; a.ld16 = 0; a.cond_len = cond_len;
    a.kw_table = kw_table; a.kw_len = kw_len; a.kw_pitch = kw_pitch;
    a.q_groups = q_groups; a.qg_pitch = qg_pitch; a.k_groups = k_groups; a.kg_pitch = kg_pitch;
    return launch_attention(a, (hipStream_t)stream);
}
extern "C" int paella_op_attention_ragged(const float* q, const float* k_self, const float* v_self, const float* k_cond, const float* v_cond,
                                          float* out, int B, int nhead, int D, int Lq, int Lself, int Lcond, const int* cond_len, const float* key_weights,
                                          int n_kw, void* stream) {
    return op_attention_impl(q, k_self, v_self, k_cond, v_cond, out, B, nhead, D, Lq, Lself, Lcond, cond_len, key_weights, n_kw, nullptr, nullptr, 0, nullptr, 0, nullptr, 0, stream);
}
extern "C" int paella_op_attention_kw(const float* q, const float* k_self, const float* v_self, const float* k_cond, const float* v_cond, float* out, int B, int nhead,
                                      int D, int Lq, int Lself, int Lcond, const int* cond_len, const float* kw_table, const int* kw_len, int kw_pitch, void* stream) {
    return op_attention_impl(q, k_self, v_self, k_cond, v_cond, out, B, nhead, D, Lq, Lself, Lcond, cond_len, nullptr, 0, kw_table, kw_len, kw_pitch, nullptr, 0, nullptr, 0, stream);
}
extern "C" int paella_op_attention_rg(const float* q, const float* k_self, const float* v_self, const float* k_cond, const float* v_cond, float* out, int B, int nhead,
                                      int D, int Lq, int Lself, int Lcond, const int* cond_len, const float* kw_table, const int* kw_len, int kw_pitch,
                                      const int* q_groups, int qg_pitch, const int* k_groups, int kg_pitch, void* stream) {
    return op_attention_impl(q, k_self, v_self, k_cond, v_cond, out, B, nhead, D, Lq, Lself, Lcond, cond_len, nullptr, 0, kw_table, kw_len, kw_pitch, q_groups, qg_pitch,
                             k_groups, kg_pitch, stream);
}
extern "C" int paella_op_attention(const float* q, const float* k_self, const float* v_self, const float* k_cond, const float* v_cond,
                                   float* out, int B, int nhead, int D, int Lq, int Lself, int Lcond, const float* key_weights,
                                   int n_kw, void* stream) {
    return paella_op_attention_ragged(q, k_self, v_self, k_cond, v_cond, out, B, nhead, D, Lq, Lself, Lcond, nullptr, key_weights, n_kw, stream);
}
static int test_attention_bf16_impl(const unsigned short* q16, const unsigned short* ks16, const unsigned short* vs16, const float* k_cond, const float* v_cond,
                                    unsigned short* out16, int B, int nhead, int D, int Lq, int Lself, int Lcond, const int* cond_len, const float* key_weights,
                                    int n_kw, const float* kw_table, const int* kw_len, int kw_pitch, void* stream) {
    AttnArgs a;
    const int ld = nhead * D;
    a.q = nullptr; a.ldq = ld; a.k_self = nullptr; a.v_self = nullptr; a.ld_self = ld; a.k_cond = k_cond; a.v_cond = v_cond; a.ld_cond = ld;
    a.out = nullptr; a.ldo = ld; a.B = B; a.nhead = nhead; a.D = D; a.Lq = Lq; a.Lself = Lself; a.Lcond = Lcond;
    a.scale = 1.0f / sqrtf((float)D); a.key_weights = key_weights; a.n_kw = key_weights ? n_kw : 0; a.out16 = out16;
    a.q16 = q16; a.k_self16 = ks16; a.v_self16 = vs16; a.ld16 = ld; a.cond_len = cond_len;
// ... 18 lines not shown
```

paella_amd/csrc/vqmodel.hip:

```cpp
#include "internal.h"
#include "../../include/paella_hip.h"

#include <math.h>
#include <stdio.h>

#include <map>
#include <string>
#include <vector>

enum VqOp { VQ_CONV1, VQ_RES, VQ_CONV4S2, VQ_CONVT4, VQ_LATENT_BN };

struct VqBlock {
    VqOp op;
    int c_in, c_out;
    Weight *w = nullptr, *b = nullptr;
    Weight *dw_w = nullptr, *dw_b = nullptr, *w1 = nullptr, *b1 = nullptr, *w2 = nullptr, *b2 = nullptr, *gammas = nullptr;
    Weight *bn_w = nullptr, *bn_b = nullptr, *bn_mean = nullptr, *bn_var = nullptr;
    float gam[6];
    DevBuf phase_w[4];
};

struct paella_vqgan {
    paella_vqgan_config cfg;
    std::vector<int> c_levels;
// ... 138 lines not shown
    hipStream_t st = (hipStream_t)stream;
    for (auto& kv : v->t)
        if (!kv.second.w.loaded) { paella_set_error("tensor '%s' was never loaded", kv.first.c_str()); return PAELLA_ERR_STATE; }
    HIP_CHECK_RET(hipStreamSynchronize(st));
    for (auto* seq : {&v->enc, &v->dec})
        for (auto& b : *seq) {
            if (b.op == VQ_RES) {
                HIP_CHECK_RET(hipMemcpy(b.gam, b.gammas->w.p, 6 * sizeof(float), hipMemcpyDeviceToHost));
            } else if (b.op == VQ_CONVT4) {
                const float* w4 = b.w->w.p;
                for (int ph = 0; ph < 4; ++ph) {
                    const int py = ph >> 1, px = ph & 1;
                    RET_IF(devbuf_alloc(b.phase_w[ph], (size_t)b.c_out * 4 * b.c_in));
                    for (int tap = 0; tap < 4; ++tap) {
                        const int ty = tap >> 1, tx = tap & 1;
                        const int ky = py == 0 ? (ty == 0 ? 1 : 3) : (ty == 0 ? 0 : 2);
                        const int kx = px == 0 ? (tx == 0 ? 1 : 3) : (tx == 0 ? 0 : 2);
                        RET_IF(launch_copy_rows(w4 + ((size_t)(ky * 4 + kx) * b.c_out) * b.c_in, b.c_in, b.phase_w[ph].p + tap * b.c_in,
                                                4 * b.c_in, b.c_out, b.c_in, st));
                    }
                }
            } else if (b.op == VQ_LATENT_BN) {
                const int cl = v->cfg.c_latent;
                std::vector<float> w(cl), bb(cl), mu(cl), var(cl), sc(cl), sh(cl);
                HIP_CHECK_RET(hipMemcpy(w.data(), b.bn_w->w.p, cl * sizeof(float), hipMemcpyDeviceToHost));
                HIP_CHECK_RET(hipMemcpy(bb.data(), b.bn_b->w.p, cl * sizeof(float), hipMemcpyDeviceToHost));
                HIP_CHECK_RET(hipMemcpy(mu.data(), b.bn_mean->w.p, cl * sizeof(float), hipMemcpyDeviceToHost));
                HIP_CHECK_RET(hipMemcpy(var.data(), b.bn_var->w.p, cl * sizeof(float), hipMemcpyDeviceToHost));
                for (int i = 0; i < cl; ++i) {
                    const float inv = 1.0f / sqrtf(var[i] + v->bn_eps);
                    sc[i] = w[i] * inv;
                    sh[i] = bb[i] - mu[i] * sc[i];
                }
                RET_IF(devbuf_alloc(v->bn_scale, cl));
                RET_IF(devbuf_alloc(v->bn_shift, cl));
                HIP_CHECK_RET(hipMemcpy(v->bn_scale.p, sc.data(), cl * sizeof(float), hipMemcpyHostToDevice));
                HIP_CHECK_RET(hipMemcpy(v->bn_shift.p, sh.data(), cl * sizeof(float), hipMemcpyHostToDevice));
            }
        }
    HIP_CHECK_RET(hipStreamSynchronize(st));
    v->finalized = true;
    if (v->precision == 1) RET_IF(vq_make_shadows(v, st));
    return PAELLA_OK;
}

extern "C" int paella_vqgan_set_precision(paella_vqgan* v, int mode, void* stream) {
    if (!v) { paella_set_error("null argument"); return PAELLA_ERR_ARG; }
    if (mode != 0 && mode != 1) { paella_set_error("precision mode must be 0 (fp32) or 1 (bf16 operands)"); return PAELLA_ERR_ARG; }
    v->precision = mode;
    if (mode == 1 && v->finalized) return vq_make_shadows(v, (hipStream_t)stream);
    return PAELLA_OK;
}

struct VqBuffers { float *x, *t, *g, *a, *lat, *qe, *splitk; unsigned short *t16, *g16; };

static void vq_carve(const paella_vqgan* v, Arena& a, int B, int h, int w, VqBuffers& f) {
    f.splitk = a.take(kSplitKBudget / sizeof(float));
    const int L = v->cfg.levels;
    size_t xmax = 0, amax = 0;
    for (int i = 0; i < L; ++i) {
        const size_t rows = (size_t)B * (h << (L - 1 - i)) * (w << (L - 1 - i));
        const size_t n = rows * v->c_levels[i];
        if (n > xmax) xmax = n;
        if (i + 1 < L) {
            const size_t r1 = (size_t)B * (h << (L - 2 - i)) * (w << (L - 2 - i));
            const size_t a1 = r1 * 4 * v->c_levels[i + 1], a2 = r1 * 16 * v->c_levels[i];
            if (a1 > amax) amax = a1;
            if (a2 > amax) amax = a2;
        }
    }
    const size_t img_rows = (size_t)B * (h << (L - 1)) * (w << (L - 1));
    if (img_rows * 12 > amax) amax = img_rows * 12;
    f.x = a.take(xmax);
    f.t = a.take(xmax);
    f.g = a.take(4 * xmax);
    f.a = a.take(amax ? amax : 4);
    f.lat = a.take((size_t)B * h * w * v->cfg.c_latent);
    f.qe = a.take((size_t)B * h * w * v->cfg.c_latent);
    f.t16 = f.g16 = nullptr;
    if (v->precision == 1) {
        f.t16 = reinterpret_cast<unsigned short*>(a.take(xmax / 2 + 64));
        f.g16 = reinterpret_cast<unsigned short*>(a.take(2 * xmax + 64));
    }
}

extern "C" size_t paella_vqgan_workspace_bytes(const paella_vqgan* v, int B, int h, int w) {
    if (!v) return 0;
    VqBuffers f;
    Arena a(nullptr, 0);
    vq_carve(v, a, B, h, w, f);
    return a.off + 256;
}

static int vq_resblock(const paella_vqgan* v, const VqBlock& b, VqBuffers& f, int B, int h, int w, hipStream_t st) {
    const int c = b.c_in;
    const int64_t rows = (int64_t)B * h * w;
    RET_IF(launch_layernorm(f.x, f.t, rows, c, 1e-6f, 1.0f + b.gam[0], b.gam[1], 0, 0, 0, st));
    RET_IF(launch_dwconv_res(f.x, f.t, b.dw_w->w.p, b.dw_b->w.p, f.x, B, h, w, c,
                             b.gam[2], st));
    const unsigned short* const w1_16 = VW16(v, b.w1);
    const unsigned short* const w2_16 = VW16(v, b.w2);
    if (w1_16 && w2_16 && f.t16 && (c % 64) == 0) {
        RET_IF(launch_layernorm16(f.x, nullptr, f.t16, rows, c, 1e-6f, 1.0f + b.gam[3], b.gam[4], 0, 0, 0, st));
        GemmArgs g1 = gemm_args(nullptr, c, b.w1->w.p, c, nullptr, 4 * c, (int)rows, 4 * c, c);
        g1.A16 = f.t16; g1.W16 = w1_16;
        g1.ep.bias = b.b1->w.p;
        g1.ep.act = ACT_GELU;
        g1.ep.c16 = f.g16;
        RET_IF(launch_gemm(g1, f.splitk, kSplitKBudget, st));
        GemmArgs g2 = gemm_args(nullptr, 4 * c, b.w2->w.p, 4 * c, f.x, c, (int)rows, c, 4 * c);
        g2.A16 = f.g16; g2.W16 = w2_16;
        g2.ep.bias = b.b2->w.p;
        g2.ep.alpha = b.gam[5];
        g2.ep.residual = f.x; g2.ep.ldr = c;
        RET_IF(launch_gemm(g2, f.splitk, kSplitKBudget, st));
        return PAELLA_OK;
    }
    RET_IF(launch_layernorm(f.x, f.t, rows, c, 1e-6f, 1.0f + b.gam[3], b.gam[4], 0, 0, 0, st));
    GemmArgs g1 = gemm_args(f.t, c, b.w1->w.p, c, f.g, 4 * c, (int)rows, 4 * c, c);
    g1.ep.bias = b.b1->w.p;
    g1.ep.act = ACT_GELU;
    RET_IF(launch_gemm(g1, f.splitk, kSplitKBudget, st));
    GemmArgs g2 = gemm_args(f.g, 4 * c, b.w2->w.p, 4 * c, f.x, c, (int)rows, c, 4 * c);
    g2.ep.bias = b.b2->w.p;
    g2.ep.alpha = b.gam[5];
    g2.ep.residual = f.x; g2.ep.ldr = c;
    RET_IF(launch_gemm(g2, f.splitk, kSplitKBudget, st));
    return PAELLA_OK;
}

static int vq_run_decoder(paella_vqgan* v, VqBuffers& f, int B, int h, int w, float* img_out, hipStream_t st) {
    int ch = h, cw = w;
    const float* in = f.lat;
    for (VqBlock& b : v->dec) {
        const int64_t rows = (int64_t)B * ch * cw;
        switch (b.op) {
            case VQ_CONV1: {
                GemmArgs g = gemm_args(in, b.c_in, b.w->w.p, b.c_in, f.x, b.c_out, (int)rows, b.c_out, b.c_in);
                g.ep.bias = b.b->w.p;
                RET_IF(launch_gemm(g, f.splitk, kSplitKBudget, st));
                break;
            }
            case VQ_RES: RET_IF(vq_resblock(v, b, f, B, ch, cw, st)); break;
            case VQ_CONVT4: {
                for (int ph = 0; ph < 4; ++ph) {
                    const int py = ph >> 1, px = ph & 1;
                    const bool implicit = (b.c_in & 31) == 0;
                    if (!implicit) RET_IF(launch_convT4_gather(f.x, f.a, B, ch, cw, b.c_in, py, px, st));
                    GemmArgs g = gemm_args(implicit ? f.x : f.a, 4 * b.c_in, b.phase_w[ph].p, 4 * b.c_in, f.t, b.c_out, (int)rows, b.c_out, 4 * b.c_in);
                    if (implicit) {
                        g.cv.enabled = 1; g.cv.Hi = ch; g.cv.Wi = cw; g.cv.C = b.c_in; g.cv.Ho = ch; g.cv.Wo = cw; g.cv.stride = 1; g.cv.ntaps = 4;
                        g.cv.tw_log2 = 1; g.cv.oy0 = py; g.cv.ox0 = px; g.cv.tsign = -1;
                    }
                    g.ep.bias = b.b->w.p;
                    g.ep.store_mode = STORE_D2S; g.ep.sH = ch; g.ep.sW = cw; g.ep.sC = b.c_out; g.ep.n_seg_x = 1; g.ep.py = py; g.ep.px = px;
                    RET_IF(launch_gemm(g, f.splitk, kSplitKBudget, st));
                }
                float* tmp = f.x; f.x = f.t; f.t = tmp;
                ch <<= 1; cw <<= 1;
                break;
            }
            default: break;
        }
    }
    const int64_t rows = (int64_t)B * ch * cw;
    GemmArgs g = gemm_args(f.x, v->c_levels[0], v->out_w->w.p, v->c_levels[0], img_out, 4, (int)rows, 12, v->c_levels[0]);
    g.ep.bias = v->out_b->w.p;
    g.ep.store_mode = STORE_PIXSHUF_NCHW; g.ep.sH = ch; g.ep.sW = cw; g.ep.sC = 3;
    RET_IF(launch_gemm(g, f.splitk, kSplitKBudget, st));
    return PAELLA_OK;
}

// ... 123 lines not shown
```

paella_amd/modules.py:

```python
import ctypes
import itertools
import math

import torch
from torch import nn
from torch.nn.modules import module as _nn_module

from . import _lib
from .training import TRAIN_SWITCHES

_TRAIN_SWITCH = {sw.name: sw for sw in TRAIN_SWITCHES}


_REGISTRATIONS = [0]
_LOAD_GENS = itertools.count(1)


def _count_registration(module, name, value):
    _REGISTRATIONS[0] += 1


_nn_module.register_module_parameter_registration_hook(_count_registration)
_nn_module.register_module_buffer_registration_hook(_count_registration)
_nn_module.register_module_module_registration_hook(_count_registration)
# ... 524 lines not shown
                raise ValueError("%d conditioning rows do not fit a slot of %d rows" % (S, slot_rows))
            self._check_table(lens_out, (B,), torch.int32, "lens_out")
        with torch.cuda.device(dev):
            nbytes = lib.paella_unet_cond_bytes(h, B, S if slot_rows is None else slot_rows)
            if out is None:
                buf = torch.empty(int(nbytes), dtype=torch.uint8, device=dev)
            elif out.device != dev or out.dtype != torch.uint8 or not out.is_contiguous() or out.numel() != int(nbytes):
                raise ValueError("out must be a contiguous uint8 tensor of %d bytes on the model's device" % int(nbytes))
            else:
                buf = out
            ws = self._workspace(lib.paella_unet_workspace_bytes(h, B, 0, 0, S), ws)
            if slot_rows is not None:
                _lib.check(lib.paella_unet_cond_prepare_slots(h, _lib.ptr(byt5) if Sb > 0 else None, Sb, _lib.ptr(clip), arr, len(images), B, slot_rows, 0,
                                                              _lib.ptr(buf), buf.numel(), _lib.ptr(lens_out), _lib.ptr(ws), ws.numel(), _lib.stream_ptr(dev)))
                return CondCache(buf, B, slot_rows, lens_out, gen=self._load_gen)
            _lib.check(lib.paella_unet_cond_prepare(h, _lib.ptr(byt5) if Sb > 0 else None, Sb, _lib.ptr(clip), arr, len(images), B,
                                                    _lib.ptr(buf), buf.numel(), _lib.ptr(ws), ws.numel(), _lib.stream_ptr(dev)))
        return CondCache(buf, B, S, gen=self._load_gen)

    def _check_cond(self, cond):
        gen = getattr(cond, "gen", None)
        if gen is not None and gen != self._load_gen:
            raise RuntimeError("this CondCache holds K/V computed from other weights: the module's weights changed (and were reloaded) after prepare_cond, or the "
                               "cache was prepared by another module -- call prepare_cond again")

    def _cond_lens(self, cond):
        lens = getattr(cond, "lens", None)
        if lens is not None:
            self._check_table(lens, (cond.B,), torch.int32, "CondCache.lens")
        return lens

    def gen_c_embeddings(self, byt5, clip, clip_image):
        h = self._engine()
        lib = _lib.load()
        dev = self._device()
        byt5, clip, images, arr, B, Sb, S = self._cond_args(byt5, clip, clip_image)
        out = torch.empty(B, S, self.c_cond, dtype=torch.float32, device=dev)
        with torch.cuda.device(dev):
            ws = self._workspace(lib.paella_unet_workspace_bytes(h, B, 0, 0, S))
            _lib.check(lib.paella_unet_c_embeddings(h, _lib.ptr(byt5) if Sb > 0 else None, Sb, _lib.ptr(clip), arr, len(images), B,
                                                    _lib.ptr(out), _lib.ptr(ws), ws.numel(), _lib.stream_ptr(dev)))
        return out

    def gen_r_embedding(self, r, max_positions=10000):
        h = self._engine()
        dev = self._device()
        r = self._f32(r, "r")
        out = torch.empty(r.numel(), self.c_r, dtype=torch.float32, device=dev)
        with torch.cuda.device(dev):
            _lib.check(_lib.load().paella_unet_r_embedding(h, _lib.ptr(r), r.numel(), float(max_positions), _lib.ptr(out),
                                                           _lib.stream_ptr(dev)))
        return out

    def forward_prepared(self, x, r, cond, attn_weights=None, out=None, cfg_mix=None, ws=None, req_mix=None, regions=None):
        return self._forward_prepared_raw(x, r, cond, attn_weights=attn_weights, out=out, cfg_mix=cfg_mix, ws=ws, req_mix=req_mix, regions=regions).permute(0, 3, 1, 2)

    def _forward_prepared_raw(self, x, r, cond, attn_weights=None, out=None, cfg_mix=None, ws=None, req_mix=None, regions=None):
        h = self._engine()
        lib = _lib.load()
        dev = self._device()
        if not x.is_cuda or x.dtype != torch.int64 or x.dim() != 3:
            raise ValueError("x must be an int64 HIP tensor [B, H, W]")
        x = x.contiguous()
        nu, H, W = x.shape
        r = self._f32(r, "r")
        if r.numel() != nu:
            raise ValueError("r must have one entry per sample")
        self._check_cond(cond)
        B = cond.B
        if nu <= 0 or B % nu:
            raise ValueError("conditioning batch %d is not a multiple of the token batch %d" % (B, nu))
        aw, kw = self._key_weights(attn_weights, B)
        rg = self._regions(regions, B, H, W, cond.S)
        if rg is not None and aw is not None:
            raise ValueError("regions take prompt weights as a KeyWeights table, not as one attn_weights vector")
        mix = (0.0, 0.0) if cfg_mix is None else (float(cfg_mix[0]), float(cfg_mix[1]))
        if cfg_mix is not None and (B != 2 * nu or mix == (0.0, 0.0)):
            raise ValueError("cfg_mix needs a conditioning batch of twice the token batch and a non-zero mix")
        if req_mix is not None:
            if cfg_mix is not None or B != 2 * nu:
                raise ValueError("req_mix needs a conditioning batch of twice the token batch and no cfg_mix")
            self._check_table(req_mix, (nu, 2), torch.float32, "req_mix")
        Bo = nu if (cfg_mix is not None or req_mix is not None) else B
        if out is None:
            out = torch.empty(Bo, H, W, self.num_labels, dtype=torch.float32, device=dev)
        elif tuple(out.shape) != (Bo, H, W, self.num_labels) or out.dtype != torch.float32 or not out.is_contiguous():
            raise ValueError("out must be a contiguous fp32 [B,H,W,num_labels] tensor")
        lens = self._cond_lens(cond)
        with torch.cuda.device(dev):
            ws = self._workspace(lib.paella_unet_workspace_bytes(h, B, H, W, cond.S), ws)
            pairs = req_mix
            if (kw is not None or rg is not None) and cfg_mix is not None:
                if torch.cuda.is_current_stream_capturing():
                    raise ValueError("forward_prepared with a KeyWeights table turns cfg_mix into a pair table by a host-to-device copy, which a graph capture "
                                     "cannot hold: pass req_mix (an fp32 device tensor [Bx, 2]) instead of cfg_mix inside a capture")
                pairs, mix = torch.tensor([mix] * nu, dtype=torch.float32).to(dev), (0.0, 0.0)
            s = self._step_block(x, r, cond, mix, pairs, lens, aw, kw, rg)
            s.logits_out = out.data_ptr()
            _lib.check(lib.paella_unet_step(h, ctypes.byref(s), ctypes.sizeof(s), _lib.ptr(ws), ws.numel(), _lib.stream_ptr(dev)))
        return out

    @staticmethod
    def _step_block(x, r, cond, mix, pairs, lens, aw, kw, rg):
        s = _lib.StepArgs(B=cond.B, n_unique=x.size(0), mix_c=mix[0], mix_u=mix[1], H=x.size(1), W=x.size(2), S=cond.S, n_attn_weights=0 if aw is None else aw.numel())
        _lib.tensor_fields(s, tokens=x, r=r, cond=cond.buf, mix_pairs=pairs, cond_len=lens, attn_weights=aw)
        if kw is not None:
            _lib.tensor_fields(s, kw_table=kw.buf, kw_len=kw.lens).kw_pitch = kw.pitch
        if rg is not None:
            _lib.tensor_fields(s, q_groups=rg.q_groups, k_groups=rg.k_groups)
            s.qg_pitch, s.kg_pitch = rg.q_groups.size(1), rg.k_groups.size(1)
        return s

    def forward_sample(self, x, r, cond, out, *, temperature, argmax=False, seed=0, seed_dev=None, offset=0, row_offset=0,
                       row_offset_dev=None, init_noise=None, t_next=0.0, cfg_mix=None, attn_weights=None, ws=None, req=None, stream=None, pin=None, regions=None):
        h = self._engine()
        lib = _lib.load()
        dev = self._device()
        if not x.is_cuda or x.dtype != torch.int64 or x.dim() != 3:
            raise ValueError("x must be an int64 HIP tensor [B, H, W]")
        x = x.contiguous()
        nu, H, W = x.shape
        r = self._f32(r, "r")
        self._check_cond(cond)
        B = cond.B
        mix = (0.0, 0.0) if cfg_mix is None else (float(cfg_mix[0]), float(cfg_mix[1]))
        if req is not None:
            seeds, temps, pairs = req
            if argmax or cfg_mix is not None or B != (nu if pairs is None else 2 * nu):
                raise ValueError("forward_sample(req=...) is categorical, takes its guidance from the pair table and needs cond.B == Bx (no pairs) or 2*Bx")
            self._check_table(seeds, (nu,), torch.int64, "req seeds")
            self._check_table(temps, (nu,), torch.float32, "req temperature")
            if pairs is not None:
                self._check_table(pairs, (nu, 2), torch.float32, "req pairs")
            if stream is not None:
                if init_noise is None:
                    raise ValueError("forward_sample(stream=...) needs init_noise: it is the renoise source of every slot")
                self._check_table(stream[0], (nu,), torch.int32, "stream step")
                self._check_table(stream[1], (nu,), torch.float32, "stream t_next")
                self._check_table(stream[2], (nu,), torch.int32, "stream active")
        elif stream is not None:
            raise ValueError("forward_sample(stream=...) needs the request tables (req=...)")
        elif (cfg_mix is None and B != nu) or (cfg_mix is not None and (B != 2 * nu or mix == (0.0, 0.0))):
            raise ValueError("forward_sample needs cond.B == Bx (no guidance) or cond.B == 2*Bx with a non-zero cfg_mix")
        if tuple(out.shape) != (nu, H, W) or out.dtype != torch.int64 or not out.is_contiguous():
            raise ValueError("out must be a contiguous int64 [B,H,W] tensor")
        if pin is not None:
            if argmax or (req is not None and stream is None) or len(pin) != (2 if stream is None else 3):
                raise ValueError("forward_sample(pin=...) is categorical and takes (keep, known), or (keep, known, pin_on) together with stream=...; "
                                 "it is not offered with req=... alone")
            self._check_table(pin[0], (nu, H, W), torch.int64, "pin keep")
            self._check_table(pin[1], (nu, H, W), torch.int64, "pin known")
            if stream is not None:
                self._check_table(pin[2], (nu,), torch.int32, "pin pin_on")
        aw, kw = self._key_weights(attn_weights, B, one_d=False)
        if kw is not None and req is None:
            raise ValueError("forward_sample takes a KeyWeights table for attn_weights only with the request tables (req=...); the scalar form takes one 1-D vector")
        rg = self._regions(regions, B, H, W, cond.S)
        if rg is not None and (stream is None or aw is not None):
            raise ValueError("forward_sample takes regions only with the stream tables (stream=...), and prompt weights next to them as a KeyWeights table")
        lens = self._cond_lens(cond)
        with torch.cuda.device(dev):
            ws = self._workspace(lib.paella_unet_workspace_bytes(h, B, H, W, cond.S), ws)
            t = _lib.TailArgs(offset=int(offset), t_next=float(t_next))
            _lib.tensor_fields(t, init_noise=init_noise, tokens_out=out)
            if req is None:
                t.temperature, t.mode, t.seed, t.row_offset = float(temperature), 1 if argmax else 0, int(seed), int(row_offset)
                _lib.tensor_fields(t, seed_ptr=seed_dev, row_offset_ptr=row_offset_dev)
            else:
                _lib.tensor_fields(t, seeds=seeds, temperature_tab=temps).rows_per_sample = H * W
            if stream is not None:
                _lib.tensor_fields(t, step=stream[0], t_next_tab=stream[1], active=stream[2])
            if pin is not None:
                _lib.tensor_fields(t, pin_keep=pin[0], pin_tokens=pin[1], pin_on=None if stream is None else pin[2])
            s = self._step_block(x, r, cond, mix, None if req is None else pairs, lens, aw, kw, rg)
            s.tail = ctypes.pointer(t)
            _lib.check(lib.paella_unet_step(h, ctypes.byref(s), ctypes.sizeof(s), _lib.ptr(ws), ws.numel(), _lib.stream_ptr(dev)))
        return out

    def forward(self, x, r, byt5, clip=None, clip_image=None, x_cat=None, **kwargs):
        unknown = set(kwargs) - {"attn_weights"}
        if unknown:
            raise TypeError("unsupported attention kwargs: %s" % sorted(unknown))
        if self.training:
            from .training import forward_autograd
            return forward_autograd(self, x, r, byt5, clip, clip_image, x_cat, kwargs.get("attn_weights"))
        if x_cat is not None:
            x = torch.cat([x, x_cat], dim=1)
        cond = self.prepare_cond(byt5, clip, clip_image)
        run_base = lambda: self._forward_prepared_raw(x, r, cond, attn_weights=kwargs.get("attn_weights"))
        run = lambda: run_base().permute(0, 3, 1, 2)
        if torch.is_grad_enabled():
            anchor = getattr(self, "_grad_anchor", None)
            if anchor is None or not anchor.requires_grad:
                anchor = next((p for p in self.parameters() if p.requires_grad), None)
                object.__setattr__(self, "_grad_anchor", anchor)
            if anchor is not None:
                return _InferenceOnly.apply(anchor, run_base).permute(0, 3, 1, 2)
        return run()

    def forward_loss(self, x, r, target, byt5, clip=None, clip_image=None, x_cat=None, attn_weights=None, label_smoothing=0.1, seeds=None):
        if not self.training:
            raise RuntimeError("forward_loss is the training path and this module is in eval mode: call model.train() first (eval mode serves the HIP inference engine)")
        from .training import forward_loss
        return forward_loss(self, x, r, target, byt5, clip, clip_image, x_cat, attn_weights, label_smoothing, seeds)

    def add_noise(self, x, t, mask=None, random_x=None):
        self._require_hip()
        dev = x.device
        if not x.is_cuda or x.dtype != torch.int64:
            raise ValueError("x must be an int64 HIP tensor")
        x = x.contiguous()
        B = x.size(0)
        per = x.numel() // max(B, 1)
        rand_u = None
        if mask is None:
            rand_u = torch.rand_like(x.float())
            t = self._f32(t, "t")
            if t.numel() != B:
                raise ValueError("t must have one entry per sample")
        else:
            mask = mask.to(torch.int64).expand_as(x).contiguous()
        if random_x is None:
            random_x = torch.randint_like(x, 0, self.num_labels)
        random_x = random_x.to(torch.int64).expand_as(x).contiguous()
        x_out = torch.empty_like(x)
        mask_out = torch.empty_like(x)
        with torch.cuda.device(dev):
# ... 15 lines not shown
```

paella_amd/sampling.py:

```python
import ctypes

import torch

from . import _lib
from ._graph import GraphOwner
from .modules import MAX_REGIONS, CondCache, KeyWeights, Paella, RegionTables, region_query_groups, region_query_total


def linspace_schedule(start, end, n):
    return [float(v) for v in torch.linspace(start, end, n)]


def _same_cond_layout(a, b):
    if a is None or b is None:
        return False
    for k in ("byt5", "clip", "clip_image"):
        va, vb = a.get(k), b.get(k)
        if (va is None) != (vb is None):
            return False
        if va is None:
            continue
        if isinstance(va, (list, tuple)) != isinstance(vb, (list, tuple)):
            return False
        if isinstance(va, (list, tuple)):
# ... 360 lines not shown
        kw.set(b, c)
        if guided:
            kw.set(B + b, u)
    return kw


def _request_keys(model, H, W, model_inputs, unconditional_inputs):
    return (min_attention_keys(model._cfg, H, W, _cond_seq_len(model, model_inputs)),
            min_attention_keys(model._cfg, H, W, _cond_seq_len(model, unconditional_inputs)) if unconditional_inputs is not None else None)


def timestep_table(t_list, steps, B, device):
    return torch.tensor([float(v) for v in t_list[:steps]], dtype=torch.float32).to(device)[:, None].repeat(1, B).contiguous()


def select_tokens(a, b=None, mask=None, flag=None, fill=-1, out=None):
    dev = a.device
    if dev.type != "cuda" or a.dtype != torch.int64:
        raise ValueError("select_tokens needs int64 HIP tensors")
    a = a.contiguous()
    for name, t in (("b", b), ("mask", mask)):
        if t is not None and (t.dtype != torch.int64 or t.shape != a.shape or t.device != dev):
            raise ValueError("select_tokens: %s must be an int64 tensor of a's shape on a's device" % name)
    if flag is not None and (flag.dtype != torch.float32 or flag.numel() != 1 or flag.device != dev):
        raise ValueError("select_tokens: flag must be a 1-element fp32 tensor on a's device")
    if out is None:
        out = torch.empty_like(a)
    with torch.cuda.device(dev):
        _lib.check(_lib.load().paella_select_tokens(_lib.ptr(a), _lib.ptr(None if b is None else b.contiguous()), _lib.ptr(None if mask is None else mask.contiguous()),
                                                    _lib.ptr(flag), int(fill), a.numel(), _lib.ptr(out), _lib.stream_ptr(dev)))
    return out


def _sample_core(model, model_inputs, unconditional_inputs, latent_shape, init_x, steps, renoise_steps, t_list, temperatures,
                 cfgs, device, noise="torch", seed=None, attn_weights=None, seed_dev=None, init_noise_buf=None, r_all=None, shard=None,
                 ws=None, fused_tail=True, row_offset_dev=None, req=None, pin=None, filt=None, conf=None):
    device = torch.device(device)
    B, H, W = shape = tuple(int(v) for v in latent_shape)
    L = model.num_labels
    native = isinstance(model, Paella)
    _refuse_core_args(noise, device, native, shape, temperatures[:steps], init_x, shard, req, pin)
    philox = noise == "philox"
    if seed is None:
        seed = fresh_seed() if philox and seed_dev is None else 0
    row_offset = 0 if shard is None else int(shard[0]) * H * W
    with torch.inference_mode():
        init_noise = _start_noise(noise, L, shape, seed, device, shard, req, init_noise_buf, seed_dev, row_offset_dev)
        sampled = init_noise.clone() if init_x is None else init_x.to(device=device, dtype=torch.int64).contiguous()
        cond_c, cond_u, cond_both, batched = _prepare_conditioning(model, model_inputs, unconditional_inputs, B, cfgs, philox, ws) if native else (None, None, None, False)
        bufs = {}
        out = torch.empty(B, H, W, dtype=torch.int64, device=device)
        if r_all is None:
            r_all = timestep_table(t_list, steps, B, device)
        fuse = philox and native and fused_tail and filt is None and conf is None
        stats = None if conf is None else tuple(torch.empty(B, H, W, dtype=torch.float32, device=device) for _ in range(2))
        for i in range(steps):
            cfg, temp = cfgs[i], temperatures[i]
            t_next = t_list[i + 1] if i < renoise_steps else None
            if fuse and (cfg is None or (batched and temp != 0)):
                model.forward_sample(sampled, r_all[i], cond_c if cfg is None else cond_both, out, temperature=temp if temp != 0 else 1.0, argmax=temp == 0,
                                     seed=seed, seed_dev=seed_dev, offset=i, row_offset=row_offset, row_offset_dev=row_offset_dev,
                                     init_noise=None if t_next is None else init_noise, t_next=0.0 if t_next is None else t_next,
                                     cfg_mix=cfg if req is None else None, attn_weights=attn_weights, ws=ws,
                                     req=None if req is None else req.step(i), **({} if pin is None else {"pin": pin}))
            else:
                lc, lu = _step_logits(model, sampled, r_all[i], i, cfg, philox and temp != 0, (cond_c, cond_u, cond_both, batched), bufs,
                                      (model_inputs, unconditional_inputs), attn_weights, ws, req)
                noise_q, mask_u = _step_noise(noise, i, shape, L, device, temp != 0, t_next is not None)
                _draw(lc, lu, out, i, temp, cfg, t_next, init_noise, (seed, seed_dev, row_offset, row_offset_dev), noise_q, mask_u, req, pin, filt, conf, stats)
            sampled = out
    if conf is not None and req is None and conf[2]:
        return sampled, {"logprob": stats[0], "entropy": stats[1]}
    return sampled


def _refuse_core_args(noise, device, native, shape, temperatures, init_x, shard, req, pin):
    explicit = isinstance(noise, dict)
    if not explicit and noise not in ("torch", "philox"):
        raise ValueError("noise must be 'torch', 'philox' or a dict of explicit noise tensors")
    if device.type != "cuda":
        raise RuntimeError("paella_amd.sample runs on a HIP device only (got device=%s); there is no CPU path" % device)
    _lib.load()
    philox = noise == "philox"
    if shard is not None and not (philox or explicit):
        raise ValueError("shard=(lo, total) needs noise='philox' (or explicit noise tensors): torch's generator stream cannot be sharded")
    if req is not None and not (philox and native and shard is None and init_x is None):
        raise ValueError("a request batch needs noise='philox', a paella_amd.Paella model, no shard and no init_x")
    if pin is not None:
        if not philox or req is not None:
            raise ValueError("pin=(keep, known) needs noise='philox' (the counter-based sampling tail re-imposes the known tokens) and no request tables")
        if any(t == 0 for t in temperatures):
            raise ValueError("pin=(keep, known) is not offered with a step temperature of 0 (the argmax extension)")
        for name, t in zip(("keep", "known"), pin):
            if not torch.is_tensor(t) or t.dtype != torch.int64 or tuple(t.shape) != shape or t.device.type != "cuda" or not t.is_contiguous():
                raise ValueError("pin: %s must be a contiguous int64 HIP tensor of shape %s" % (name, shape))


def _start_noise(noise, L, shape, seed, device, shard, req, buf, seed_dev, row_offset_dev):
    if req is not None:
        return start_tokens_requests(L, shape, req.seeds, out=buf)
    if noise == "philox":
        return start_tokens(L, shape, seed, device, shard, out=buf, seed_dev=seed_dev, row_offset_dev=row_offset_dev)
    if buf is not None:
        return buf
    if isinstance(noise, dict):
        return noise["init_noise"].to(device=device, dtype=torch.int64).contiguous()
    return torch.randint(0, L, size=shape, device=device)


def _prepare_conditioning(model, model_inputs, unconditional_inputs, B, cfgs, philox, ws):
    any_cfg = any(c is not None for c in cfgs)
    cond_c = cond_u = cond_both = None
    if any_cfg and _same_cond_layout(model_inputs, unconditional_inputs):
        cond_both = model.prepare_cond(**_cat_inputs(model_inputs, unconditional_inputs), ws=ws)
    elif any_cfg and philox and _cond_batch(model_inputs) == B and _cond_batch(unconditional_inputs) == B \
            and min(_cond_seq_len(model, model_inputs), _cond_seq_len(model, unconditional_inputs)) > 0:
        cond_both = _prepare_ragged_pair(model, model_inputs, unconditional_inputs, B, ws)
    batched = cond_both is not None
    if not batched or not all(c is not None for c in cfgs):
        cond_c = model.prepare_cond(**model_inputs, ws=ws)
        cond_u = model.prepare_cond(**unconditional_inputs, ws=ws) if any_cfg and not batched else None
    return cond_c, cond_u, cond_both, batched


def _step_logits(model, sampled, r, i, cfg, fold, conds, bufs, inputs, attn_weights, ws, req):
    cond_c, cond_u, cond_both, batched = conds
    B, H, W = sampled.shape

    def logits_buf(name, rows_b):
        if name not in bufs:
            bufs[name] = torch.empty(rows_b, H, W, model.num_labels, dtype=torch.float32, device=sampled.device)
        return bufs[name]
    if not isinstance(model, Paella):
        lc = model(sampled, r, **inputs[0]).permute(0, 2, 3, 1).float().contiguous()
        return lc, (model(sampled, r, **inputs[1]).permute(0, 2, 3, 1).float().contiguous() if cfg is not None else None)
    if cfg is not None and batched:
        logits2 = logits_buf("both", 2 * B)
        model.forward_prepared(sampled, r, cond_both, attn_weights=attn_weights, out=logits2[:B] if fold else logits2,
                               cfg_mix=cfg if fold and req is None else None, ws=ws, **({} if req is None else {"req_mix": req.pairs[i]}))
        return logits2[:B], (None if fold else logits2[B:])
    lc, lu = logits_buf("c", B), None
    model.forward_prepared(sampled, r, cond_c, attn_weights=attn_weights, out=lc, ws=ws)
    if cfg is not None:
        lu = logits_buf("u", B)
        model.forward_prepared(sampled, r, cond_u, attn_weights=attn_weights, out=lu, ws=ws)
    return lc, lu


def _step_noise(noise, i, shape, L, device, categorical, renoise):
    if noise == "philox":
        return None, None
    if isinstance(noise, dict):
        given = lambda t: t.to(device=device, dtype=torch.float32).contiguous()
        return given(noise["q"][i]) if categorical else None, given(noise["u"][i]) if renoise else None
    B, H, W = shape
    rows = B * H * W
    noise_q = mask_u = None
    if categorical:
        if B == 1:
            noise_q = torch.empty(L, rows, dtype=torch.float32, device=device).exponential_(1).t().contiguous()
        else:
            noise_q = torch.empty(rows, L, dtype=torch.float32, device=device).exponential_(1)
    if renoise:
        mask_u = torch.rand(B, H, W, dtype=torch.float32, device=device)
    return noise_q, mask_u


def _draw(lc, lu, out, i, temp, cfg, t_next, init_noise, words, noise_q, mask_u, req, pin, filt, conf, stats):
    rows, L = out.numel(), lc.size(-1)
    hw = rows // out.size(0)
    renoise = t_next is not None
    seed, seed_dev, row_offset, row_offset_dev = words
    cfg, omc = (1.0, 0.0) if cfg is None else cfg
    if conf is not None and req is not None:
        _stream_draw(lc, lu, rows, L, out, (None if lu is None else req.pairs[i], req.temps[i], req.seeds, hw), filt.step[i], filt.t_next[i] if renoise else None,
                     filt.active, init_noise, (filt.k, filt.mass), conf=(conf.never, conf.policy, conf.noise, *stats), renoise=renoise)
    elif conf is not None:
        _run_tail(lc, lu, rows, L, out, scalar=(cfg, omc, temp, 0, seed, seed_dev, row_offset, row_offset_dev, None, None), offset=i, pin=None if renoise else pin,
                  filt=FILTER_OFF if filt is None else filt, stats=stats)
        if renoise:
            _renoise_stage(out, stats[0], init_noise, rows, hw, seed, i, t_next, conf[0], conf[1], out, seed_dev=seed_dev, row_offset=row_offset,
                           row_offset_dev=row_offset_dev, pin=pin)
    elif req is not None:
        _tail_req(lc, lu, rows, L, hw, req, i, init_noise if renoise or filt is not None else None, t_next if renoise else 0.0, out, filt=filt)
    else:
        _tail(lc, lu, rows, L, cfg, omc, temp if temp != 0 else 1.0, int(temp == 0), noise_q, seed, i, init_noise if renoise else None, mask_u,
              t_next if renoise else 0.0, out, seed_dev=seed_dev, row_offset=row_offset, row_offset_dev=row_offset_dev, pin=pin, filt=filt)


def _call_filter(noise, temperatures, top_k, top_p, typical_mass, min_tokens):
    f = check_filter(top_k, top_p, typical_mass, min_tokens)
    if not filter_on(f):
        return None
    _philox_only(_filter_names(top_k, top_p, typical_mass), "filters the draw", noise, temperatures)
    return f


def sample(model, model_inputs, latent_shape, unconditional_inputs=None, steps=12, renoise_steps=11, temperature=(1.0, 0.2),
# ... 687 lines not shown
```

Measured before the change: 47.35 images/sec.

## Precompute timestep tables for all steps and fuse several per-step seams

Computes the timestep-embedding projection for every sampling step in one launch before the loop and passes each step's row into the UNet step. The aim is to drop the per-step timestep kernel. It also adds a fused depthwise-conv+residual+layernorm kernel, a layernorm-then-CFG-mix kernel, a multi-segment replicate kernel and a VQ front path, all gated by a seam mask that defaults to all on. These remove several small launches and intermediate round-trips per step, at the cost of more code paths and an extra table buffer.

New measurement: 47.59 images/sec (median of 6 runs). About the same (+0.5%).

```diff
diff --git a/include/paella_hip.h b/include/paella_hip.h
--- a/include/paella_hip.h
+++ b/include/paella_hip.h
@@ -237,7 +237,11 @@
     const float* kw_table; const int32_t* kw_len; int32_t kw_pitch;
     const int32_t* q_groups; int32_t qg_pitch; const int32_t* k_groups; int32_t kg_pitch;
     float* logits_out; const paella_tail_args* tail;
+    const float* ts_pre; int32_t ts_pre_rows;
 } paella_step_args;
+
+size_t paella_unet_timestep_table_floats(const paella_unet* m, int S, int B_ts);
+int paella_unet_timestep_tables(paella_unet* m, const float* r, int S, int n_unique, int B_ts, float* ts_out, float* remb_out, void* stream);
 
 int paella_unet_step(paella_unet* m, const paella_step_args* args, size_t args_bytes, void* ws, size_t ws_bytes, void* stream);
 int paella_sample_tail_args(const paella_tail_args* args, size_t args_bytes, void* stream);
diff --git a/paella_amd/_lib.py b/paella_amd/_lib.py
--- a/paella_amd/_lib.py
+++ b/paella_amd/_lib.py
@@ -66,6 +66,7 @@
         ("kw_table", c_void_p), ("kw_len", c_void_p), ("kw_pitch", c_int32),
         ("q_groups", c_void_p), ("qg_pitch", c_int32), ("k_groups", c_void_p), ("kg_pitch", c_int32),
         ("logits_out", c_void_p), ("tail", POINTER(TailArgs)),
+        ("ts_pre", c_void_p), ("ts_pre_rows", c_int32),
     ]
 
 
@@ -100,6 +101,8 @@
     "paella_unet_c_embeddings": (c_int, [c_void_p, c_void_p, c_int, c_void_p, POINTER(c_void_p), c_int, c_int, c_void_p,
                                          c_void_p, c_size_t, c_void_p]),
     "paella_unet_r_embedding": (c_int, [c_void_p, c_void_p, c_int, c_float, c_void_p, c_void_p]),
+    "paella_unet_timestep_table_floats": (c_size_t, [c_void_p, c_int, c_int]),
+    "paella_unet_timestep_tables": (c_int, [c_void_p, c_void_p, c_int, c_int, c_int, c_void_p, c_void_p, c_void_p]),
     "paella_unet_forward": (c_int, [c_void_p, c_void_p, c_void_p, c_void_p, c_int, c_int, c_int, c_int, c_void_p, c_int,
                                     c_void_p, c_void_p, c_size_t, c_void_p]),
     "paella_unet_forward_shared": (c_int, [c_void_p, c_void_p, c_void_p, c_void_p, c_int, c_int, c_float, c_float, c_int, c_int, c_int,
@@ -292,6 +295,11 @@
     "paella_test_gemm_desc": (c_int, [POINTER(TestGemmArgs), c_int, c_int, c_void_p, c_size_t, c_void_p]),
     "paella_test_gemm_args_size": (c_size_t, []),
     "paella_test_embed_ln_unshuffle": (c_int, [c_void_p, c_void_p, c_void_p, c_int, c_int, c_int, c_int, c_int, c_int, c_float, c_void_p]),
+    "paella_test_step_seams": (c_int, [c_int]),
+    "paella_test_replicate_segs": (c_int, [POINTER(c_void_p), POINTER(c_void_p), POINTER(c_int64), c_int, c_int, c_void_p]),
+    "paella_test_copy_rows": (c_int, [c_void_p, c_void_p, c_int64, c_int, c_void_p]),
+    "paella_test_layernorm_mix": (c_int, [c_void_p, c_void_p, c_int64, c_int, c_float, c_float, c_int, c_void_p]),
+    "paella_test_vq_front": (c_int, [c_void_p, c_void_p, c_void_p, c_void_p, c_void_p, c_void_p, c_int, c_int, c_int, c_int, c_float, c_float, c_float, c_int, c_void_p]),
 }
 
 _lib = None
diff --git a/paella_amd/csrc/common.h b/paella_amd/csrc/common.h
--- a/paella_amd/csrc/common.h
+++ b/paella_amd/csrc/common.h
@@ -165,6 +165,7 @@
                      int s2d, int H, int W, hipStream_t stream);
 int launch_layernorm16(const float* x, float* y, unsigned short* y16, int64_t rows, int C, float eps, float g_mul, float g_add,
                        int s2d, int H, int W, hipStream_t stream);
+int launch_layernorm_mix(const float* x, float* out, int64_t rows_half, int C, float eps, float a, float b, hipStream_t stream);
 int launch_grn_apply16(unsigned short* h, const float* scale, const float* shift, int64_t rows, int rows_per_sample, int C, hipStream_t stream);
 int launch_grn_partials_apply16(const float* part, const float* gamma, const float* shift, float* scale, unsigned short* h, int B, int rows_per_sample, int C, hipStream_t stream);
 int launch_f32_to_bf16(const float* src, unsigned short* dst, size_t n, hipStream_t stream);
@@ -175,6 +176,9 @@
 int launch_dwconv_res(const float* x, const float* xt, const float* w, const float* bias, float* y,
                       int B, int H, int W, int C, float gamma2, hipStream_t stream);
 
+int launch_dwconv_res_ln(const float* x, const float* xt, const float* w, const float* bias, float* y, float* t, unsigned short* t16,
+                         int B, int H, int W, int C, float gamma2, float eps, float g_mul, float g_add, hipStream_t stream);
+
 int launch_grn_scale(const float* g, const float* gamma, float* scale, float* tmp_gx, int B,
                      int rows_per_sample, int C, hipStream_t stream);
 
@@ -185,11 +189,17 @@
 
 int launch_timestep(const float* r, const float* freqs, const float* Wcat, const float* bcat, float* ts,
                     int B, int c_r, int total, float max_positions, float* r_embed_out, int reps, hipStream_t stream);
+int launch_timestep_steps(const float* r, const float* freqs, const float* Wcat, const float* bcat, float* ts, int S,
+                          int B, int c_r, int total, float max_positions, float* r_embed_out, int reps, hipStream_t stream);
 int launch_scale_shift(float* x, const float* ts, int ts_stride, int64_t rows, int rows_per_sample, int C,
                        hipStream_t stream);
 
 int launch_silu(const float* x, float* y, int64_t n, hipStream_t stream);
 int launch_copy_rows(const float* src, int lds, float* dst, int ldd, int64_t rows, int cols, hipStream_t stream);
+struct ReplicateSegs { const float* src[4]; float* dst[4]; int64_t n[4]; unsigned blk_end[4]; int nseg; };
+int launch_replicate_segs(ReplicateSegs segs, int reps, hipStream_t stream);
+enum { kSeamTimestep = 1, kSeamReplicate = 2, kSeamLnMix = 4, kSeamVqFront = 8, kSeamAll = 15 };
+int step_seams();
 int launch_axpby(float* x, const float* y, float a, float b, int64_t n, hipStream_t stream);
 int launch_axpby16(float* x, const float* y, float a, float b, int64_t n, unsigned short* x16, hipStream_t stream);
 int launch_axpby16_req(float* x, const float* y, const float* ab, int B, int64_t per_sample, unsigned short* x16, hipStream_t stream);
diff --git a/paella_amd/csrc/elementwise.hip b/paella_amd/csrc/elementwise.hip
--- a/paella_amd/csrc/elementwise.hip
+++ b/paella_amd/csrc/elementwise.hip
@@ -105,6 +105,40 @@
     const unsigned blocks = (unsigned)((rows + WAVES_PER_BLOCK - 1) / WAVES_PER_BLOCK);
     DISPATCH_NV(C >> 2, hipLaunchKernelGGL((layernorm_kernel<NV>), dim3(blocks), dim3(64 * WAVES_PER_BLOCK), 0, st, x, y, y16,
                                            rows, C, eps, g_mul, g_add, s2d, H, W));
+    LAUNCH_CHECK_RET();
+    return PAELLA_OK;
+}
+
+template <int NV>
+__global__ __launch_bounds__(64 * WAVES_PER_BLOCK) void layernorm_mix_kernel(const float* __restrict__ x, float* __restrict__ out, int64_t rows_half, int C, float eps,
+                                                                            float g_mul, float g_add, float a, float b) {
+    const int lane = threadIdx.x & 63;
+    const int64_t row = (int64_t)blockIdx.x * WAVES_PER_BLOCK + (threadIdx.x >> 6);
+    if (row >= rows_half) return;
+    const int C4 = C >> 2;
+    f32x4 vc[NV], vu[NV];
+    const float* xc = x + row * C;
+    const float* xu = x + (rows_half + row) * C;
+#pragma unroll
+    for (int i = 0; i < NV; ++i) {
+        const int c4 = lane + i * 64;
+        vc[i] = c4 < C4 ? ld4(xc + c4 * 4) : f32x4{0.f, 0.f, 0.f, 0.f};
+        vu[i] = c4 < C4 ? ld4(xu + c4 * 4) : f32x4{0.f, 0.f, 0.f, 0.f};
+    }
+    ln_regs<NV>(vc, C4, lane, C, eps, g_mul, g_add);
+    ln_regs<NV>(vu, C4, lane, C, eps, g_mul, g_add);
+#pragma unroll
+    for (int i = 0; i < NV; ++i) {
+        const int c4 = lane + i * 64;
+        if (c4 < C4) st4(out + row * C + c4 * 4, vc[i] * a + vu[i] * b);
+    }
+}
+
+int launch_layernorm_mix(const float* x, float* out, int64_t rows_half, int C, float eps, float a, float b, hipStream_t st) {
+    if (rows_half <= 0) return PAELLA_OK;
+    if (C & 3) { paella_set_error("layernorm_mix: C %% 4 != 0 (C=%d)", C); return PAELLA_ERR_ARG; }
+    const unsigned blocks = (unsigned)((rows_half + WAVES_PER_BLOCK - 1) / WAVES_PER_BLOCK);
+    DISPATCH_NV(C >> 2, hipLaunchKernelGGL((layernorm_mix_kernel<NV>), dim3(blocks), dim3(64 * WAVES_PER_BLOCK), 0, st, x, out, rows_half, C, eps, 1.f, 0.f, a, b));
     LAUNCH_CHECK_RET();
     return PAELLA_OK;
 }
@@ -204,6 +238,80 @@
     return PAELLA_OK;
 }
 
+template <int NV>
+__global__ __launch_bounds__(64 * WAVES_PER_BLOCK) void dwconv_res_ln_kernel(const float* __restrict__ x, const float* __restrict__ xt, const float* __restrict__ w,
+                                                                            const float* __restrict__ bias, float* __restrict__ y, float* __restrict__ t,
+                                                                            unsigned short* __restrict__ t16, int B, int H, int W, int C, float gamma2, float eps,
+                                                                            float g_mul, float g_add) {
+    const int lane = threadIdx.x & 63;
+    const int64_t pos = (int64_t)blockIdx.x * WAVES_PER_BLOCK + (threadIdx.x >> 6);
+    const int64_t total = (int64_t)B * H * W;
+    if (pos >= total) return;
+    const int C4 = C >> 2;
+    const int xx = (int)(pos % W);
+    const int yy = (int)((pos / W) % H);
+    const int64_t base = pos - (int64_t)yy * W - xx;
+    f32x4 acc[NV];
+#pragma unroll
+    for (int i = 0; i < NV; ++i) {
+        const int c4 = lane + i * 64;
+        acc[i] = c4 < C4 ? ld4(bias + c4 * 4) : f32x4{0.f, 0.f, 0.f, 0.f};
+    }
+#pragma unroll
+    for (int ky = 0; ky < 3; ++ky) {
+        const int sy = min(max(yy + ky - 1, 0), H - 1);
+#pragma unroll
+        for (int kx = 0; kx < 3; ++kx) {
+            const int sx = min(max(xx + kx - 1, 0), W - 1);
+            const int64_t npos = base + (int64_t)sy * W + sx;
+            const int tap = ky * 3 + kx;
+#pragma unroll
+            for (int i = 0; i < NV; ++i) {
+                const int c4 = lane + i * 64;
+                if (c4 < C4) acc[i] += ld4(xt + npos * C + c4 * 4) * ld4(w + tap * C + c4 * 4);
+            }
+        }
+    }
+#pragma unroll
+    for (int i = 0; i < NV; ++i) {
+        const int c4 = lane + i * 64;
+        if (c4 < C4) {
+            acc[i] = ld4(x + pos * C + c4 * 4) + acc[i] * gamma2;
+            st4(y + pos * C + c4 * 4, acc[i]);
+        } else {
+            acc[i] = f32x4{0.f, 0.f, 0.f, 0.f};
+        }
+    }
+    ln_regs<NV>(acc, C4, lane, C, eps, g_mul, g_add);
+    if (t16) {
+#pragma unroll
+        for (int i = 0; i < NV; ++i) {
+            const int c4 = lane + i * 64;
+            if (c4 < C4) st4h(t16 + pos * C + c4 * 4, acc[i]);
+        }
+    }
+    if (t) {
+#pragma unroll
+        for (int i = 0; i < NV; ++i) {
+            const int c4 = lane + i * 64;
+            if (c4 < C4) st4(t + pos * C + c4 * 4, acc[i]);
+        }
+    }
+}
+
+int launch_dwconv_res_ln(const float* x, const float* xt, const float* w, const float* bias, float* y, float* t, unsigned short* t16, int B, int H, int W, int C,
+                         float gamma2, float eps, float g_mul, float g_add, hipStream_t st) {
+    const int64_t total = (int64_t)B * H * W;
+    if (total <= 0) return PAELLA_OK;
+    if (C & 3) { paella_set_error("dwconv_res_ln: C %% 4 != 0"); return PAELLA_ERR_ARG; }
+    if ((!t && !t16) || t == xt || t == y) { paella_set_error("dwconv_res_ln: the normalised row needs a buffer of its own (not xt, not y)"); return PAELLA_ERR_ARG; }
+    const unsigned blocks = (unsigned)((total + WAVES_PER_BLOCK - 1) / WAVES_PER_BLOCK);
+    DISPATCH_NV(C >> 2, hipLaunchKernelGGL((dwconv_res_ln_kernel<NV>), dim3(blocks), dim3(64 * WAVES_PER_BLOCK), 0, st, x, xt, w, bias, y, t, t16, B, H, W, C, gamma2,
+                                           eps, g_mul, g_add));
+    LAUNCH_CHECK_RET();
+    return PAELLA_OK;
+}
+
 __global__ __launch_bounds__(256) void grn_sumsq_kernel(const float* __restrict__ g, float* __restrict__ gx, int rows_per_sample,
                                                         int C) {
     __shared__ float red[4][64];
@@ -379,6 +487,9 @@
     extern __shared__ float emb[];
     const int b = blockIdx.y;
     const int half = c_r >> 1;
+    r += (size_t)blockIdx.z * n_distinct;
+    if (ts) ts += (size_t)blockIdx.z * reps * n_distinct * total;
+    if (r_embed_out) r_embed_out += (size_t)blockIdx.z * n_distinct * c_r;
     const float rr = r[b] * max_positions;
     for (int k = threadIdx.x; k < c_r; k += 256) {
         float v = 0.f;
@@ -399,10 +510,15 @@
 
 int launch_timestep(const float* r, const float* freqs, const float* Wcat, const float* bcat, float* ts, int B,
                     int c_r, int total, float max_positions, float* r_embed_out, int reps, hipStream_t st) {
-    if (B <= 0) return PAELLA_OK;
+    return launch_timestep_steps(r, freqs, Wcat, bcat, ts, 1, B, c_r, total, max_positions, r_embed_out, reps, st);
+}
+int launch_timestep_steps(const float* r, const float* freqs, const float* Wcat, const float* bcat, float* ts, int S, int B,
+                          int c_r, int total, float max_positions, float* r_embed_out, int reps, hipStream_t st) {
+    if (B <= 0 || S <= 0) return PAELLA_OK;
+    if (B > 65535 || S > 65535) { paella_set_error("timestep: more than 65535 samples or steps"); return PAELLA_ERR_ARG; }
     int gx = (total + 255) / 256;
     if (gx < 1) gx = 1;
-    hipLaunchKernelGGL(timestep_kernel, dim3(gx, B), dim3(256), c_r * sizeof(float), st, r, freqs, Wcat, bcat, ts, c_r,
+    hipLaunchKernelGGL(timestep_kernel, dim3(gx, B, S), dim3(256), c_r * sizeof(float), st, r, freqs, Wcat, bcat, ts, c_r,
                        total, max_positions, r_embed_out, reps < 1 ? 1 : reps, B);
     LAUNCH_CHECK_RET();
     return PAELLA_OK;
@@ -496,6 +612,49 @@
     int64_t blocks = (n / 4 + 255) / 256;
     if (blocks > 8192) blocks = 8192;
     hipLaunchKernelGGL(axpby_kernel, dim3((unsigned)blocks), dim3(256), 0, st, x, y, a, b, n / 4, x16);
+    LAUNCH_CHECK_RET();
+    return PAELLA_OK;
+}
+
+__global__ __launch_bounds__(256) void replicate_segs_kernel(ReplicateSegs s, int reps) {
+    const float* src = s.src[0];
+    float* dst = s.dst[0];
+    int64_t n = s.n[0];
+    unsigned b0 = 0, b1 = s.blk_end[0];
+#pragma unroll
+    for (int k = 1; k < 4; ++k)
+        if (k < s.nseg && blockIdx.x >= s.blk_end[k - 1]) { src = s.src[k]; dst = s.dst[k]; n = s.n[k]; b0 = s.blk_end[k - 1]; b1 = s.blk_end[k]; }
+    const int64_t first = (int64_t)(blockIdx.x - b0) * 256 + threadIdx.x, stride = (int64_t)(b1 - b0) * 256;
+    if (!((n & 3) | (((uintptr_t)src | (uintptr_t)dst) & 15))) {
+        const int64_t n4 = n >> 2;
+        for (int64_t i = first; i < n4; i += stride) {
+            const f32x4 v = ld4(src + i * 4);
+            for (int rep = 1; rep < reps; ++rep) st4(dst + (rep - 1) * n + i * 4, v);
+        }
+    } else {
+        for (int64_t i = first; i < n; i += stride) {
+            const float v = src[i];
+            for (int rep = 1; rep < reps; ++rep) dst[(rep - 1) * n + i] = v;
+        }
+    }
+}
+int launch_replicate_segs(ReplicateSegs s, int reps, hipStream_t st) {
+    if (s.nseg < 0 || s.nseg > 4) { paella_set_error("replicate: %d segments (at most 4)", s.nseg); return PAELLA_ERR_ARG; }
+    if (reps < 2) return PAELLA_OK;
+    ReplicateSegs k = {};
+    unsigned blocks = 0;
+    for (int j = 0; j < s.nseg; ++j) {
+        if (s.n[j] <= 0) continue;
+        if (!s.src[j] || !s.dst[j]) { paella_set_error("replicate: null segment"); return PAELLA_ERR_ARG; }
+        const bool v4 = !((s.n[j] & 3) | (((uintptr_t)s.src[j] | (uintptr_t)s.dst[j]) & 15));
+        int64_t b = ((v4 ? s.n[j] / 4 : s.n[j]) + 255) / 256;
+        if (b > 4096) b = 4096;
+        blocks += (unsigned)b;
+        k.src[k.nseg] = s.src[j]; k.dst[k.nseg] = s.dst[j]; k.n[k.nseg] = s.n[j]; k.blk_end[k.nseg] = blocks;
+        ++k.nseg;
+    }
+    if (!k.nseg) return PAELLA_OK;
+    hipLaunchKernelGGL(replicate_segs_kernel, dim3(blocks), dim3(256), 0, st, k, reps);
     LAUNCH_CHECK_RET();
     return PAELLA_OK;
 }
diff --git a/paella_amd/csrc/model.hip b/paella_amd/csrc/model.hip
--- a/paella_amd/csrc/model.hip
+++ b/paella_amd/csrc/model.hip
@@ -7,6 +7,7 @@
 #include <stdio.h>
 #include <string.h>
 
+#include <atomic>
 #include <map>
 #include <string>
 #include <vector>
@@ -586,6 +587,29 @@
     return launch_timestep(r, m->freqs.p, m->ts_w.p, m->ts_b.p, nullptr, B, m->cfg.c_r, 0, max_positions, r_embed_out, 1, (hipStream_t)stream);
 }
 
+static std::atomic<int> g_step_seams{kSeamAll};
+int step_seams() { return g_step_seams.load(std::memory_order_relaxed); }
+extern "C" int paella_test_step_seams(int mask) { g_step_seams = mask & kSeamAll; return PAELLA_OK; }
+
+extern "C" size_t paella_unet_timestep_table_floats(const paella_unet* m, int S, int B_ts) {
+    if (!m || S <= 0 || B_ts <= 0 || m->ts_total <= 0) return 0;
+    return (size_t)S * B_ts * m->ts_total;
+}
+extern "C" int paella_unet_timestep_tables(paella_unet* m, const float* r, int S, int n_unique, int B_ts, float* ts_out, float* remb_out, void* stream) {
+    if (!m || !m->finalized) { paella_set_error("model not finalized"); return PAELLA_ERR_STATE; }
+    if (S <= 0 || n_unique <= 0 || B_ts <= 0 || B_ts % n_unique) { paella_set_error("timestep_tables: S, n_unique > 0 and n_unique must divide B_ts"); return PAELLA_ERR_ARG; }
+    if (m->ts_total <= 0) return PAELLA_OK;
+    if (!r || !ts_out) { paella_set_error("null argument"); return PAELLA_ERR_ARG; }
+    const paella_unet_config& c = m->cfg;
+    hipStream_t st = (hipStream_t)stream;
+    if (step_seams() & kSeamTimestep)
+        return launch_timestep_steps(r, m->freqs.p, m->ts_w.p, m->ts_b.p, ts_out, S, n_unique, c.c_r, m->ts_total, 10000.0f, remb_out, B_ts / n_unique, st);
+    for (int i = 0; i < S; ++i)
+        RET_IF(launch_timestep(r + (size_t)i * n_unique, m->freqs.p, m->ts_w.p, m->ts_b.p, ts_out + (size_t)i * B_ts * m->ts_total, n_unique, c.c_r, m->ts_total, 10000.0f,
+                               remb_out ? remb_out + (size_t)i * n_unique * c.c_r : nullptr, B_ts / n_unique, st));
+    return PAELLA_OK;
+}
+
 static int cond_prepare_impl(paella_unet* m, const float* byt5, int S_byt5, const float* clip, const float* const* clip_image, int n_clip_image, int B,
                              int S_slot, int slot0, void* cond_out, size_t cond_bytes, int* cond_len, void* ws, size_t ws_bytes, void* stream) {
     if (!m || !m->finalized) { paella_set_error("model not finalized"); return PAELLA_ERR_STATE; }
@@ -829,8 +853,11 @@
         B = n_unique; cx.B = n_unique;
     }
 
-    if (m->ts_total > 0)
-        RET_IF(launch_timestep(s.r, m->freqs.p, m->ts_w.p, m->ts_b.p, f.ts, B, c.c_r, m->ts_total, 10000.0f, f.remb, Bfull / B, st));
+    if (m->ts_total > 0) {
+        if (s.ts_pre && s.ts_pre_rows < Bfull) { paella_set_error("ts_pre holds %d rows, the forward needs %d", s.ts_pre_rows, Bfull); return PAELLA_ERR_ARG; }
+        if (s.ts_pre && (step_seams() & kSeamTimestep)) f.ts = const_cast<float*>(s.ts_pre);
+        else RET_IF(launch_timestep(s.r, m->freqs.p, m->ts_w.p, m->ts_b.p, f.ts, B, c.c_r, m->ts_total, 10000.0f, f.remb, Bfull / B, st));
+    }
 
     const int h0 = H / p, w0 = W / p;
     const int64_t n0 = (int64_t)B * h0 * w0;
@@ -850,7 +877,16 @@
             const int reps = Bfull / B;
             int lvl = 0;
             for (size_t j = 0; j < bi; ++j) if (m->down[j].type == BT_DOWN) lvl = m->down[j].level;
-            for (int rep = 1; rep < reps; ++rep) {
+            const bool has_stat = f.rowstat && c.c_hidden[lvl] % 16 == 0, has_x16 = f.x16 && c.c_hidden[lvl] % 8 == 0;
+            if ((step_seams() & kSeamReplicate) && lvl + 1 + (has_stat ? 1 : 0) + (has_x16 ? 1 : 0) <= 4) {
+                ReplicateSegs sg = {};
+                auto seg = [&](float* p, int64_t n) { sg.src[sg.nseg] = p; sg.dst[sg.nseg] = p + n; sg.n[sg.nseg] = n; ++sg.nseg; };
+                for (int l = 0; l <= lvl; ++l) seg(f.xl[l], (int64_t)B * (h0 >> l) * (w0 >> l) * c.c_hidden[l]);
+                const int64_t rows_c = (int64_t)B * h * w;
+                if (has_stat) seg(f.rowstat, rows_c * (c.c_hidden[lvl] / 16 * 2));
+                if (has_x16) seg(reinterpret_cast<float*>(f.x16), rows_c * (c.c_hidden[lvl] / 2));
+                RET_IF(launch_replicate_segs(sg, reps, st));
+            } else for (int rep = 1; rep < reps; ++rep) {
                 for (int l = 0; l <= lvl; ++l) {
                     const int64_t rows_l = (int64_t)B * (h0 >> l) * (w0 >> l);
                     const int cl = c.c_hidden[l];
@@ -924,9 +960,13 @@
         RET_IF(launch_gemm(g, f.splitk, kSplitKBudget, st));
         int64_t nt = (int64_t)B * H * W;
         const unsigned short* const wh16 = (c.c_out % 64) == 0 ? W16(m, m->out_mapper) : nullptr;
-        if (wh16 && !mix) RET_IF(launch_layernorm16(f.g, nullptr, f.h16, nt, c.c_out, 1e-6f, 1.f, 0.f, 0, 0, 0, st));
+        const bool ln_mix = mix && !s.mix_pairs && !wh16 && (step_seams() & kSeamLnMix);
+        if (ln_mix) {
+            nt /= 2;
+            RET_IF(launch_layernorm_mix(f.g, f.h, nt, c.c_out, 1e-6f, s.mix_c, s.mix_u, st));
+        } else if (wh16 && !mix) RET_IF(launch_layernorm16(f.g, nullptr, f.h16, nt, c.c_out, 1e-6f, 1.f, 0.f, 0, 0, 0, st));
         else RET_IF(launch_layernorm(f.g, f.h, nt, c.c_out, 1e-6f, 1.f, 0.f, 0, 0, 0, st));
-        if (mix) {
+        if (mix && !ln_mix) {
             nt /= 2;
             if (s.mix_pairs) RET_IF(launch_axpby16_req(f.h, f.h + (size_t)nt * c.c_out, s.mix_pairs, n_unique, (int64_t)H * W * c.c_out, wh16 ? f.h16 : nullptr, st));
             else RET_IF(launch_axpby16(f.h, f.h + (size_t)nt * c.c_out, s.mix_c, s.mix_u, nt * c.c_out, wh16 ? f.h16 : nullptr, st));
@@ -1312,6 +1352,29 @@
 extern "C" int paella_test_grn_apply16(unsigned short* h, const float* scale, const float* shift, int64_t rows, int rows_per_sample, int C, void* stream) {
     return launch_grn_apply16(h, scale, shift, rows, rows_per_sample, C, (hipStream_t)stream);
 }
+extern "C" int paella_test_replicate_segs(const float* const* src, float* const* dst, const int64_t* n, int nseg, int reps, void* stream) {
+    if (nseg < 0 || nseg > 4 || !src || !dst || !n) { paella_set_error("replicate_segs: 0..4 segments"); return PAELLA_ERR_ARG; }
+    ReplicateSegs s = {};
+    for (int k = 0; k < nseg; ++k) { s.src[k] = src[k]; s.dst[k] = dst[k]; s.n[k] = n[k]; }
+    s.nseg = nseg;
+    return launch_replicate_segs(s, reps, (hipStream_t)stream);
+}
+extern "C" int paella_test_copy_rows(const float* src, float* dst, int64_t rows, int cols, void* stream) {
+    return launch_copy_rows(src, cols, dst, cols, rows, cols, (hipStream_t)stream);
+}
+extern "C" int paella_test_layernorm_mix(const float* x, float* out, int64_t rows_half, int C, float a, float b, int fused, void* stream) {
+    hipStream_t st = (hipStream_t)stream;
+    if (fused) return launch_layernorm_mix(x, out, rows_half, C, 1e-6f, a, b, st);
+    RET_IF(launch_layernorm(x, out, 2 * rows_half, C, 1e-6f, 1.f, 0.f, 0, 0, 0, st));
+    return launch_axpby16(out, out + (size_t)rows_half * C, a, b, rows_half * C, nullptr, st);
+}
+extern "C" int paella_test_vq_front(float* x, const float* xt, const float* w, const float* bias, float* t, unsigned short* t16, int B, int H, int W, int C, float gamma2,
+                                    float g_mul, float g_add, int fused, void* stream) {
+    hipStream_t st = (hipStream_t)stream;
+    if (fused) return launch_dwconv_res_ln(x, xt, w, bias, x, t, t16, B, H, W, C, gamma2, 1e-6f, g_mul, g_add, st);
+    RET_IF(launch_dwconv_res(x, xt, w, bias, x, B, H, W, C, gamma2, st));
+    return launch_layernorm16(x, t, t16, (int64_t)B * H * W, C, 1e-6f, g_mul, g_add, 0, 0, 0, st);
+}
 extern "C" int paella_op_layernorm(const float* x, float* y, int64_t rows, int C, float eps, void* stream) {
     return launch_layernorm(x, y, rows, C, eps, 1.f, 0.f, 0, 0, 0, (hipStream_t)stream);
 }
diff --git a/paella_amd/csrc/vqmodel.hip b/paella_amd/csrc/vqmodel.hip
--- a/paella_amd/csrc/vqmodel.hip
+++ b/paella_amd/csrc/vqmodel.hip
@@ -214,7 +214,7 @@
     return PAELLA_OK;
 }
 
-struct VqBuffers { float *x, *t, *g, *a, *lat, *qe, *splitk; unsigned short *t16, *g16; };
+struct VqBuffers { float *x, *t, *t2, *g, *a, *lat, *qe, *splitk; unsigned short *t16, *g16; };
 
 static void vq_carve(const paella_vqgan* v, Arena& a, int B, int h, int w, VqBuffers& f) {
     f.splitk = a.take(kSplitKBudget / sizeof(float));
@@ -244,6 +244,7 @@
         f.t16 = reinterpret_cast<unsigned short*>(a.take(xmax / 2 + 64));
         f.g16 = reinterpret_cast<unsigned short*>(a.take(2 * xmax + 64));
     }
+    f.t2 = a.take(xmax);
 }
 
 extern "C" size_t paella_vqgan_workspace_bytes(const paella_vqgan* v, int B, int h, int w) {
@@ -258,12 +259,15 @@
     const int c = b.c_in;
     const int64_t rows = (int64_t)B * h * w;
     RET_IF(launch_layernorm(f.x, f.t, rows, c, 1e-6f, 1.0f + b.gam[0], b.gam[1], 0, 0, 0, st));
-    RET_IF(launch_dwconv_res(f.x, f.t, b.dw_w->w.p, b.dw_b->w.p, f.x, B, h, w, c,
-                             b.gam[2], st));
     const unsigned short* const w1_16 = VW16(v, b.w1);
     const unsigned short* const w2_16 = VW16(v, b.w2);
-    if (w1_16 && w2_16 && f.t16 && (c % 64) == 0) {
-        RET_IF(launch_layernorm16(f.x, nullptr, f.t16, rows, c, 1e-6f, 1.0f + b.gam[3], b.gam[4], 0, 0, 0, st));
+    const bool fast = w1_16 && w2_16 && f.t16 && (c % 64) == 0;
+    const bool front = (step_seams() & kSeamVqFront) != 0;
+    if (front) RET_IF(launch_dwconv_res_ln(f.x, f.t, b.dw_w->w.p, b.dw_b->w.p, f.x, fast ? nullptr : f.t2, fast ? f.t16 : nullptr, B, h, w, c, b.gam[2], 1e-6f,
+                                           1.0f + b.gam[3], b.gam[4], st));
+    else RET_IF(launch_dwconv_res(f.x, f.t, b.dw_w->w.p, b.dw_b->w.p, f.x, B, h, w, c, b.gam[2], st));
+    if (fast) {
+        if (!front) RET_IF(launch_layernorm16(f.x, nullptr, f.t16, rows, c, 1e-6f, 1.0f + b.gam[3], b.gam[4], 0, 0, 0, st));
         GemmArgs g1 = gemm_args(nullptr, c, b.w1->w.p, c, nullptr, 4 * c, (int)rows, 4 * c, c);
         g1.A16 = f.t16; g1.W16 = w1_16;
         g1.ep.bias = b.b1->w.p;
@@ -278,8 +282,8 @@
         RET_IF(launch_gemm(g2, f.splitk, kSplitKBudget, st));
         return PAELLA_OK;
     }
-    RET_IF(launch_layernorm(f.x, f.t, rows, c, 1e-6f, 1.0f + b.gam[3], b.gam[4], 0, 0, 0, st));
-    GemmArgs g1 = gemm_args(f.t, c, b.w1->w.p, c, f.g, 4 * c, (int)rows, 4 * c, c);
+    if (!front) RET_IF(launch_layernorm(f.x, f.t, rows, c, 1e-6f, 1.0f + b.gam[3], b.gam[4], 0, 0, 0, st));
+    GemmArgs g1 = gemm_args(front ? f.t2 : f.t, c, b.w1->w.p, c, f.g, 4 * c, (int)rows, 4 * c, c);
     g1.ep.bias = b.b1->w.p;
     g1.ep.act = ACT_GELU;
     RET_IF(launch_gemm(g1, f.splitk, kSplitKBudget, st));
diff --git a/paella_amd/modules.py b/paella_amd/modules.py
--- a/paella_amd/modules.py
+++ b/paella_amd/modules.py
@@ -600,10 +600,33 @@
                                                            _lib.stream_ptr(dev)))
         return out
 
-    def forward_prepared(self, x, r, cond, attn_weights=None, out=None, cfg_mix=None, ws=None, req_mix=None, regions=None):
-        return self._forward_prepared_raw(x, r, cond, attn_weights=attn_weights, out=out, cfg_mix=cfg_mix, ws=ws, req_mix=req_mix, regions=regions).permute(0, 3, 1, 2)
-
-    def _forward_prepared_raw(self, x, r, cond, attn_weights=None, out=None, cfg_mix=None, ws=None, req_mix=None, regions=None):
+    def timestep_tables(self, r_all, B_ts):
+        h = self._engine()
+        lib = _lib.load()
+        dev = self._device()
+        if not torch.is_tensor(r_all) or r_all.dim() != 2 or r_all.dtype != torch.float32 or not r_all.is_cuda or not r_all.is_contiguous():
+            raise ValueError("r_all must be a contiguous fp32 HIP tensor [steps, B]")
+        S, nu = r_all.shape
+        if S <= 0 or nu <= 0 or B_ts <= 0 or B_ts % nu:
+            raise ValueError("timestep_tables: B_ts (%d) must be a positive multiple of the token batch (%d)" % (B_ts, nu))
+        n = int(lib.paella_unet_timestep_table_floats(h, S, B_ts))
+        if n == 0:
+            return None
+        with torch.cuda.device(dev):
+            out = torch.empty(S, B_ts, n // (S * B_ts), dtype=torch.float32, device=dev)
+            _lib.check(lib.paella_unet_timestep_tables(h, _lib.ptr(r_all), S, nu, B_ts, _lib.ptr(out), None, _lib.stream_ptr(dev)))
+        return out
+
+    def _check_ts_pre(self, ts_pre, B):
+        if ts_pre is not None and (not torch.is_tensor(ts_pre) or ts_pre.dim() != 2 or ts_pre.dtype != torch.float32 or not ts_pre.is_cuda or not ts_pre.is_contiguous()
+                                   or ts_pre.size(0) < B):
+            raise ValueError("ts_pre must be one step's row of timestep_tables: a contiguous fp32 HIP tensor [>= %d, ts_total]" % B)
+
+    def forward_prepared(self, x, r, cond, attn_weights=None, out=None, cfg_mix=None, ws=None, req_mix=None, regions=None, ts_pre=None):
+        return self._forward_prepared_raw(x, r, cond, attn_weights=attn_weights, out=out, cfg_mix=cfg_mix, ws=ws, req_mix=req_mix, regions=regions,
+                                          ts_pre=ts_pre).permute(0, 3, 1, 2)
+
+    def _forward_prepared_raw(self, x, r, cond, attn_weights=None, out=None, cfg_mix=None, ws=None, req_mix=None, regions=None, ts_pre=None):
         h = self._engine()
         lib = _lib.load()
         dev = self._device()
@@ -643,13 +666,14 @@
                     raise ValueError("forward_prepared with a KeyWeights table turns cfg_mix into a pair table by a host-to-device copy, which a graph capture "
                                      "cannot hold: pass req_mix (an fp32 device tensor [Bx, 2]) instead of cfg_mix inside a capture")
                 pairs, mix = torch.tensor([mix] * nu, dtype=torch.float32).to(dev), (0.0, 0.0)
-            s = self._step_block(x, r, cond, mix, pairs, lens, aw, kw, rg)
+            self._check_ts_pre(ts_pre, B)
+            s = self._step_block(x, r, cond, mix, pairs, lens, aw, kw, rg, ts_pre)
             s.logits_out = out.data_ptr()
             _lib.check(lib.paella_unet_step(h, ctypes.byref(s), ctypes.sizeof(s), _lib.ptr(ws), ws.numel(), _lib.stream_ptr(dev)))
         return out
 
     @staticmethod
-    def _step_block(x, r, cond, mix, pairs, lens, aw, kw, rg):
+    def _step_block(x, r, cond, mix, pairs, lens, aw, kw, rg, ts_pre=None):
         s = _lib.StepArgs(B=cond.B, n_unique=x.size(0), mix_c=mix[0], mix_u=mix[1], H=x.size(1), W=x.size(2), S=cond.S, n_attn_weights=0 if aw is None else aw.numel())
         _lib.tensor_fields(s, tokens=x, r=r, cond=cond.buf, mix_pairs=pairs, cond_len=lens, attn_weights=aw)
         if kw is not None:
@@ -657,10 +681,13 @@
         if rg is not None:
             _lib.tensor_fields(s, q_groups=rg.q_groups, k_groups=rg.k_groups)
             s.qg_pitch, s.kg_pitch = rg.q_groups.size(1), rg.k_groups.size(1)
+        if ts_pre is not None:
+            _lib.tensor_fields(s, ts_pre=ts_pre).ts_pre_rows = ts_pre.size(0)
         return s
 
     def forward_sample(self, x, r, cond, out, *, temperature, argmax=False, seed=0, seed_dev=None, offset=0, row_offset=0,
-                       row_offset_dev=None, init_noise=None, t_next=0.0, cfg_mix=None, attn_weights=None, ws=None, req=None, stream=None, pin=None, regions=None):
+                       row_offset_dev=None, init_noise=None, t_next=0.0, cfg_mix=None, attn_weights=None, ws=None, req=None, stream=None, pin=None, regions=None,
+                       ts_pre=None):
         h = self._engine()
         lib = _lib.load()
         dev = self._device()
@@ -720,7 +747,8 @@
                 _lib.tensor_fields(t, step=stream[0], t_next_tab=stream[1], active=stream[2])
             if pin is not None:
                 _lib.tensor_fields(t, pin_keep=pin[0], pin_tokens=pin[1], pin_on=None if stream is None else pin[2])
-            s = self._step_block(x, r, cond, mix, None if req is None else pairs, lens, aw, kw, rg)
+            self._check_ts_pre(ts_pre, B)
+            s = self._step_block(x, r, cond, mix, None if req is None else pairs, lens, aw, kw, rg, ts_pre)
             s.tail = ctypes.pointer(t)
             _lib.check(lib.paella_unet_step(h, ctypes.byref(s), ctypes.sizeof(s), _lib.ptr(ws), ws.numel(), _lib.stream_ptr(dev)))
         return out
diff --git a/paella_amd/sampling.py b/paella_amd/sampling.py
--- a/paella_amd/sampling.py
+++ b/paella_amd/sampling.py
@@ -436,6 +436,10 @@
         out = torch.empty(B, H, W, dtype=torch.int64, device=device)
         if r_all is None:
             r_all = timestep_table(t_list, steps, B, device)
+        ts_all = None
+        if native and req is None and steps > 0:
+            ts_all = model.timestep_tables(r_all[:steps].contiguous(), 2 * B if batched and any(c is not None for c in cfgs[:steps]) else B)
+        ts_step = (lambda i: None) if ts_all is None else (lambda i: ts_all[i])
         fuse = philox and native and fused_tail and filt is None and conf is None
         stats = None if conf is None else tuple(torch.empty(B, H, W, dtype=torch.float32, device=device) for _ in range(2))
         for i in range(steps):
@@ -446,10 +450,10 @@
                                      seed=seed, seed_dev=seed_dev, offset=i, row_offset=row_offset, row_offset_dev=row_offset_dev,
                                      init_noise=None if t_next is None else init_noise, t_next=0.0 if t_next is None else t_next,
                                      cfg_mix=cfg if req is None else None, attn_weights=attn_weights, ws=ws,
-                                     req=None if req is None else req.step(i), **({} if pin is None else {"pin": pin}))
+                                     req=None if req is None else req.step(i), ts_pre=ts_step(i), **({} if pin is None else {"pin": pin}))
             else:
                 lc, lu = _step_logits(model, sampled, r_all[i], i, cfg, philox and temp != 0, (cond_c, cond_u, cond_both, batched), bufs,
-                                      (model_inputs, unconditional_inputs), attn_weights, ws, req)
+                                      (model_inputs, unconditional_inputs), attn_weights, ws, req, ts_step(i))
                 noise_q, mask_u = _step_noise(noise, i, shape, L, device, temp != 0, t_next is not None)
                 _draw(lc, lu, out, i, temp, cfg, t_next, init_noise, (seed, seed_dev, row_offset, row_offset_dev), noise_q, mask_u, req, pin, filt, conf, stats)
             sampled = out
@@ -507,7 +511,7 @@
     return cond_c, cond_u, cond_both, batched
 
 
-def _step_logits(model, sampled, r, i, cfg, fold, conds, bufs, inputs, attn_weights, ws, req):
+def _step_logits(model, sampled, r, i, cfg, fold, conds, bufs, inputs, attn_weights, ws, req, ts_pre=None):
     cond_c, cond_u, cond_both, batched = conds
     B, H, W = sampled.shape
 
@@ -521,13 +525,13 @@
     if cfg is not None and batched:
         logits2 = logits_buf("both", 2 * B)
         model.forward_prepared(sampled, r, cond_both, attn_weights=attn_weights, out=logits2[:B] if fold else logits2,
-                               cfg_mix=cfg if fold and req is None else None, ws=ws, **({} if req is None else {"req_mix": req.pairs[i]}))
+                               cfg_mix=cfg if fold and req is None else None, ws=ws, ts_pre=ts_pre, **({} if req is None else {"req_mix": req.pairs[i]}))
         return logits2[:B], (None if fold else logits2[B:])
     lc, lu = logits_buf("c", B), None
-    model.forward_prepared(sampled, r, cond_c, attn_weights=attn_weights, out=lc, ws=ws)
+    model.forward_prepared(sampled, r, cond_c, attn_weights=attn_weights, out=lc, ws=ws, ts_pre=ts_pre)
     if cfg is not None:
         lu = logits_buf("u", B)
-        model.forward_prepared(sampled, r, cond_u, attn_weights=attn_weights, out=lu, ws=ws)
+        model.forward_prepared(sampled, r, cond_u, attn_weights=attn_weights, out=lu, ws=ws, ts_pre=ts_pre)
     return lc, lu
 
 
```
